# sidiso/surfh

Measured on AMD Instinct MI355X. Metric: CG-iterations/sec (forward+adjoint) on 251x251x4000 cube, higher is better.
Workload: dtype f32 (storage and accumulation; products as 2-piece fp16 splits -- 3 products per fp32 product, 1 on the far tails of the spectral response -- on the 16-bit matrix cores, in the spectral-blur GEMM and in the DFT passes)

## Files before the change

### include/surfh_amd.h

```cpp
#ifndef SURFH_AMD_H
#define SURFH_AMD_H

#include <stdint.h>

#ifdef __cplusplus
extern "C" {
#endif

typedef struct surfh_plan surfh_plan;

typedef struct {
    int32_t wslice_start, wslice_stop;
    int32_t n_pointings;
    int32_t n_slit;
    int32_t n_lambda_out;
    int32_t n_alpha_out;
    int32_t srf;
    int32_t na, nb;
    int32_t alpha0;
    int32_t n_alpha_slit;
    int32_t n_beta_slit;
    const int32_t *slit_beta0;
    const double *slit_weights;
    const int32_t *grid_i0;
    const int32_t *grid_i1;
    const double *grid_y0;
    const double *grid_y1;
    const double *wpsf;
    const int32_t *gt_i0;
    const int32_t *gt_i1;
    const double *gt_y0;
    const double *gt_y1;
    const uint8_t *gt_inside;
    int32_t box_len, box_shift;
} surfh_channel_desc;

typedef struct {
    int32_t n_alpha, n_beta;
    int32_t n_lambda;
    int32_t n_templates;
    const double *templates;
    const double *sotf;
    int32_t n_channels;
    const surfh_channel_desc *channels;
    int32_t device;
    void *stream;
    int32_t split_k_forward;
    int32_t verify;
    int32_t exact;
} surfh_config;

const char *surfh_last_error(void);
int surfh_version(void);

int surfh_plan_create(const surfh_config *cfg, surfh_plan **out);
int surfh_plan_destroy(surfh_plan *plan);

int64_t surfh_isize(const surfh_plan *plan);
int64_t surfh_osize(const surfh_plan *plan);
void *surfh_stream(const surfh_plan *plan);

int surfh_forward(surfh_plan *plan, const float *maps, float *y);
int surfh_adjoint(surfh_plan *plan, const float *y, float *maps);
int surfh_adjoint_ref(surfh_plan *plan, const float *y, float *maps);
int surfh_fwadj(surfh_plan *plan, const float *x, float *out);

int surfh_forward_dev(surfh_plan *plan, const float *maps_dev, float *y_dev);
int surfh_adjoint_dev(surfh_plan *plan, const float *y_dev, float *maps_dev);
int surfh_adjoint_ref_dev(surfh_plan *plan, const float *y_dev, float *maps_dev);
int surfh_fwadj_dev(surfh_plan *plan, const float *x_dev, float *out_dev);

int surfh_wct_forward(surfh_plan *plan, const float *maps, float *cube);
int surfh_wct_adjoint(surfh_plan *plan, const float *cube, float *maps);
int surfh_wct_fwadj(surfh_plan *plan, const float *x, float *out);
int surfh_wct_expsol(surfh_plan *plan, const float *cube, const double *mu_reg, const double *reg_freq, float *maps);

int surfh_cg(surfh_plan *plan, const float *y, double mu, double mu_reg, const float *x0,
             int32_t max_iter, double tol, int32_t refresh, float *x, double *grad_norm, int32_t *nit);
typedef int (*surfh_cg_callback)(void *user, int32_t it, const double *grad_norm, const float *x);
int surfh_cg_cb(surfh_plan *plan, const float *y, double mu, double mu_reg, const float *x0,
                int32_t max_iter, double tol, int32_t refresh, float *x, double *grad_norm, int32_t *nit,
                surfh_cg_callback callback, void *user);
int surfh_mmmg(surfh_plan *plan, const float *y, double mu, double mu_reg, const float *x0,
               int32_t max_iter, double tol, int32_t refresh, float *x, double *grad_norm, int32_t *nit,
               surfh_cg_callback callback, void *user);

int surfh_maps_to_cube(surfh_plan *plan, const double *templates, int32_t n_templates, int32_t n_lambda,
                       const float *maps, float *cube);
int surfh_cube_to_maps(surfh_plan *plan, const double *templates, int32_t n_templates, int32_t n_lambda,
                       const float *cube, float *maps);

int surfh_cg_planes(surfh_plan *plan, const float *y, double mu, double mu_reg, const float *x0, int32_t max_iter,
                    double tol, int32_t refresh, float *x, double *grad_norm, int32_t *nit);
int surfh_mmmg_planes(surfh_plan *plan, const float *y, double mu, double mu_reg, const float *x0, int32_t max_iter,
                      double tol, int32_t refresh, float *x, double *grad_norm, int32_t *nit);

int surfh_cg_planes_begin_dev(surfh_plan *plan, const float *y_dev, double mu, double mu_reg, float *x_dev);
int surfh_cg_planes_step_dev(surfh_plan *plan, int32_t iters, int32_t refresh);
int surfh_cg_planes_rr(surfh_plan *plan, double *rr_host);

int surfh_cg_planes_cb(surfh_plan *plan, const float *y, double mu, double mu_reg, const float *x0, int32_t max_iter,
                       double tol, int32_t refresh, float *x, double *grad_norm, int32_t *nit,
                       surfh_cg_callback callback, void *user);
int surfh_mmmg_planes_cb(surfh_plan *plan, const float *y, double mu, double mu_reg, const float *x0, int32_t max_iter,
                         double tol, int32_t refresh, float *x, double *grad_norm, int32_t *nit,
                         surfh_cg_callback callback, void *user);

int surfh_normal_dev(surfh_plan *plan, const float *d_dev, float *q_dev, double mu);
int surfh_prior_add_dev(surfh_plan *plan, const float *d_dev, float *q_dev, double mu_reg);
int surfh_spec_supported(surfh_plan *plan);
int64_t surfh_spec_size(surfh_plan *plan);
int surfh_to_spec_dev(surfh_plan *plan, const float *x_dev, float *xt_dev);
int surfh_from_spec_dev(surfh_plan *plan, const float *xt_dev, float *x_dev);
int surfh_forward_spec_dev(surfh_plan *plan, const float *dt_dev, float *y_dev);
int surfh_adjoint_spec_dev(surfh_plan *plan, const float *y_dev, float *qt_dev, double mu, const float *dt_dev, double mu_reg);
int surfh_normal_spec_dev(surfh_plan *plan, const float *dt_dev, float *qt_dev, double mu, double mu_reg);
int surfh_prior_spec_add_dev(surfh_plan *plan, const float *dt_dev, float *qt_dev, double mu_reg);
int surfh_set_prior(surfh_plan *plan, int32_t kind);
int surfh_dot_dev(surfh_plan *plan, const float *a_dev, const float *b_dev, int64_t n, double *out_host);
int surfh_cg_step_dev(surfh_plan *plan, float *x_dev, float *r_dev, const float *d_dev,
                      const float *q_dev, int64_t n, double rr_in, double *rr_out_host);
int surfh_cg_dir_dev(surfh_plan *plan, float *d_dev, const float *r_dev, int64_t n, double beta);
int surfh_cg_iter_dev(surfh_plan *plan, float *x_dev, float *r_dev, float *d_dev, const float *q_dev, int64_t n,
                      double rr_in, double *rr_out);

int surfh_cg_begin_dev(surfh_plan *plan, const float *r_dev, int64_t n);
int surfh_cg_iter_nosync_dev(surfh_plan *plan, float *x_dev, float *r_dev, float *d_dev, const float *q_dev, int64_t n);
int surfh_cg_xupdate_nosync_dev(surfh_plan *plan, float *x_dev, const float *d_dev, const float *q_dev, int64_t n);
int surfh_cg_refresh_nosync_dev(surfh_plan *plan, float *r_dev, const float *b_dev, const float *q_dev, float *d_dev, int64_t n);
int32_t surfh_cg_trace(surfh_plan *plan, double *out_host, int32_t capacity);
int surfh_residual_dev(surfh_plan *plan, float *r_dev, const float *b_dev, const float *q_dev, int64_t n);

int surfh_profile_enable(surfh_plan *plan, int32_t on);
int surfh_profile_filter(surfh_plan *plan, const char *prefix);
int32_t surfh_profile_count(surfh_plan *plan);
int surfh_profile_get(surfh_plan *plan, int32_t i, const char **name, int64_t *launches, double *ms);
int surfh_profile_reset(surfh_plan *plan);

int64_t surfh_debug_copy(surfh_plan *plan, const char *which, float *out, int64_t capacity);
int surfh_debug_dims(surfh_plan *plan, const char *which, int64_t dims[4]);

int surfh_gemm_selftest(int32_t device, int32_t M, int32_t N, int32_t K, int32_t split_k,
                        const float *A, const float *B, float *C);
int surfh_gemm_selftest_ksteps(int64_t near_far[2]);
int32_t surfh_klist_classify(const float *B, int32_t n, int32_t k, int64_t ldb, int32_t perm_p, int32_t perm_lin,
                             int32_t *records, int64_t capacity);

typedef struct surfh_tst surfh_tst;
int surfh_tst_create(int32_t n_alpha, int32_t n_beta, int32_t n_lambda, int32_t n_templates, const double *templates,
                     const int32_t *voxels, int64_t n_voxels, const float *S, int32_t device, surfh_tst **out);
int surfh_tst_destroy(surfh_tst *t);
int surfh_tst_forward(surfh_tst *t, const float *maps, float *cube);
int surfh_tst_adjoint(surfh_tst *t, const float *cube, float *maps);
int surfh_tst_fwadj(surfh_tst *t, const float *maps, float *out);
const char *surfh_tst_last_error(void);

int surfh_shepard(int32_t n_seg, const int64_t *pt_off, const float *pt_alpha, const float *pt_lambda,
                  const float *pt_value, const int32_t *n_alpha, const int32_t *n_lambda, int32_t separable,
                  const float *q_alpha, const float *q_lambda, const float *inv_alpha_res, const float *inv_lambda_res,
                  float p, float alpha, float pixel_cutoff, float epsilon, float *out, int32_t *neighbours,
                  int32_t device_ptrs, void *stream, float *kernel_ms);
const char *surfh_shepard_last_error(void);

#ifdef __cplusplus
}
#endif
#endif
```

### surfh_amd/_lib.py

```python
from __future__ import annotations

import ctypes as C
import os

import numpy as np

_HERE = os.path.dirname(os.path.abspath(__file__))
LIB_PATH = os.path.join(_HERE, "libsurfh_amd.so")

c_float_p = C.POINTER(C.c_float)
c_double_p = C.POINTER(C.c_double)
c_int32_p = C.POINTER(C.c_int32)
CG_CALLBACK = C.CFUNCTYPE(C.c_int, C.c_void_p, C.c_int32, c_double_p, c_float_p)
c_uint8_p = C.POINTER(C.c_uint8)


class ChannelDesc(C.Structure):
    _fields_ = [
        ("wslice_start", C.c_int32), ("wslice_stop", C.c_int32),
        ("n_pointings", C.c_int32), ("n_slit", C.c_int32), ("n_lambda_out", C.c_int32),
        ("n_alpha_out", C.c_int32), ("srf", C.c_int32), ("na", C.c_int32), ("nb", C.c_int32),
        ("alpha0", C.c_int32), ("n_alpha_slit", C.c_int32), ("n_beta_slit", C.c_int32),
        ("slit_beta0", c_int32_p), ("slit_weights", c_double_p),
        ("grid_i0", c_int32_p), ("grid_i1", c_int32_p), ("grid_y0", c_double_p), ("grid_y1", c_double_p),
        ("wpsf", c_double_p),
        ("gt_i0", c_int32_p), ("gt_i1", c_int32_p), ("gt_y0", c_double_p), ("gt_y1", c_double_p),
        ("gt_inside", c_uint8_p),
        ("box_len", C.c_int32), ("box_shift", C.c_int32),
    ]


class Config(C.Structure):
    _fields_ = [
        ("n_alpha", C.c_int32), ("n_beta", C.c_int32), ("n_lambda", C.c_int32), ("n_templates", C.c_int32),
        ("templates", c_double_p), ("sotf", c_double_p),
        ("n_channels", C.c_int32), ("channels", C.POINTER(ChannelDesc)),
        ("device", C.c_int32), ("stream", C.c_void_p), ("split_k_forward", C.c_int32), ("verify", C.c_int32),
        ("exact", C.c_int32),
    ]


EXPORTS = [
    "surfh_last_error", "surfh_version", "surfh_plan_create", "surfh_plan_destroy", "surfh_isize", "surfh_osize",
    "surfh_stream", "surfh_forward", "surfh_adjoint", "surfh_adjoint_ref", "surfh_fwadj", "surfh_forward_dev",
    "surfh_adjoint_dev", "surfh_adjoint_ref_dev", "surfh_fwadj_dev", "surfh_wct_forward", "surfh_wct_adjoint",
    "surfh_wct_fwadj", "surfh_wct_expsol", "surfh_tst_create", "surfh_tst_destroy", "surfh_tst_forward",
    "surfh_tst_adjoint", "surfh_tst_fwadj", "surfh_tst_last_error", "surfh_cg", "surfh_cg_cb", "surfh_mmmg", "surfh_cg_planes", "surfh_mmmg_planes", "surfh_cg_planes_cb", "surfh_mmmg_planes_cb", "surfh_cg_planes_begin_dev", "surfh_cg_planes_step_dev", "surfh_cg_planes_rr", "surfh_maps_to_cube", "surfh_cube_to_maps", "surfh_normal_dev",
    "surfh_prior_add_dev", "surfh_spec_supported", "surfh_spec_size", "surfh_to_spec_dev", "surfh_from_spec_dev", "surfh_forward_spec_dev",
    "surfh_adjoint_spec_dev", "surfh_normal_spec_dev", "surfh_prior_spec_add_dev", "surfh_set_prior", "surfh_dot_dev", "surfh_cg_step_dev", "surfh_cg_dir_dev", "surfh_cg_iter_dev", "surfh_residual_dev",
    "surfh_cg_begin_dev", "surfh_cg_iter_nosync_dev", "surfh_cg_xupdate_nosync_dev", "surfh_cg_refresh_nosync_dev", "surfh_cg_trace",
    "surfh_profile_enable", "surfh_profile_filter", "surfh_profile_count", "surfh_profile_get", "surfh_profile_reset", "surfh_debug_copy",
    "surfh_debug_dims", "surfh_gemm_selftest", "surfh_gemm_selftest_ksteps", "surfh_klist_classify",
    "surfh_shepard", "surfh_shepard_last_error",
]

_lib = None


def load():
    global _lib
    if _lib is not None:
        return _lib
    if not os.path.exists(LIB_PATH):
        raise RuntimeError(f"{LIB_PATH} not found: run `python -c 'import __graft_entry__ as g; g.build()'` "
                           "(the HIP path has no CPU fallback)")
    L = C.CDLL(LIB_PATH)
    vp = C.c_void_p
    L.surfh_last_error.restype = C.c_char_p
    L.surfh_version.restype = C.c_int
    L.surfh_plan_create.argtypes = [C.POINTER(Config), C.POINTER(vp)]
    L.surfh_plan_destroy.argtypes = [vp]
    L.surfh_isize.argtypes = [vp]; L.surfh_isize.restype = C.c_int64
    L.surfh_osize.argtypes = [vp]; L.surfh_osize.restype = C.c_int64
    L.surfh_stream.argtypes = [vp]; L.surfh_stream.restype = vp
    for n in ("surfh_forward", "surfh_adjoint", "surfh_adjoint_ref", "surfh_fwadj", "surfh_wct_forward", "surfh_wct_adjoint",
              "surfh_wct_fwadj"):
        getattr(L, n).argtypes = [vp, c_float_p, c_float_p]
    for n in ("surfh_forward_dev", "surfh_adjoint_dev", "surfh_adjoint_ref_dev", "surfh_fwadj_dev"):
        getattr(L, n).argtypes = [vp, vp, vp]
    L.surfh_cg.argtypes = [vp, c_float_p, C.c_double, C.c_double, c_float_p, C.c_int32, C.c_double, C.c_int32,
                           c_float_p, c_double_p, c_int32_p]
    L.surfh_tst_create.argtypes = [C.c_int32] * 4 + [c_double_p, c_int32_p, C.c_int64, c_float_p, C.c_int32, C.POINTER(vp)]
    L.surfh_tst_destroy.argtypes = [vp]
    for n in ("surfh_tst_forward", "surfh_tst_adjoint", "surfh_tst_fwadj"):
        getattr(L, n).argtypes = [vp, c_float_p, c_float_p]
    L.surfh_tst_last_error.restype = C.c_char_p
    L.surfh_wct_expsol.argtypes = [vp, c_float_p, c_double_p, c_double_p, c_float_p]
    L.surfh_cg_planes.argtypes = [vp, c_float_p, C.c_double, C.c_double, c_float_p, C.c_int32, C.c_double, C.c_int32,
                                  c_float_p, c_double_p, c_int32_p]
    L.surfh_cg_cb.argtypes = [vp, c_float_p, C.c_double, C.c_double, c_float_p, C.c_int32, C.c_double, C.c_int32,
                              c_float_p, c_double_p, c_int32_p, CG_CALLBACK, vp]
    L.surfh_mmmg.argtypes = L.surfh_cg_cb.argtypes
    L.surfh_mmmg_planes.argtypes = L.surfh_cg_planes.argtypes
    L.surfh_cg_planes_begin_dev.argtypes = [vp, vp, C.c_double, C.c_double, vp]
    L.surfh_cg_planes_step_dev.argtypes = [vp, C.c_int32, C.c_int32]
    L.surfh_cg_planes_rr.argtypes = [vp, c_double_p]
    L.surfh_cg_planes_cb.argtypes = L.surfh_cg_cb.argtypes
    L.surfh_mmmg_planes_cb.argtypes = L.surfh_cg_cb.argtypes
    L.surfh_maps_to_cube.argtypes = [vp, c_double_p, C.c_int32, C.c_int32, c_float_p, c_float_p]
    L.surfh_cube_to_maps.argtypes = [vp, c_double_p, C.c_int32, C.c_int32, c_float_p, c_float_p]
    L.surfh_normal_dev.argtypes = [vp, vp, vp, C.c_double]
    L.surfh_prior_add_dev.argtypes = [vp, vp, vp, C.c_double]
    L.surfh_spec_supported.argtypes = [vp]
    L.surfh_spec_size.argtypes = [vp]
    L.surfh_spec_size.restype = C.c_int64
    L.surfh_to_spec_dev.argtypes = [vp, vp, vp]
    L.surfh_from_spec_dev.argtypes = [vp, vp, vp]
    L.surfh_forward_spec_dev.argtypes = [vp, vp, vp]
    L.surfh_adjoint_spec_dev.argtypes = [vp, vp, vp, C.c_double, vp, C.c_double]
    L.surfh_normal_spec_dev.argtypes = [vp, vp, vp, C.c_double, C.c_double]
    L.surfh_prior_spec_add_dev.argtypes = [vp, vp, vp, C.c_double]
    L.surfh_set_prior.argtypes = [vp, C.c_int32]
    L.surfh_dot_dev.argtypes = [vp, vp, vp, C.c_int64, c_double_p]
    L.surfh_cg_step_dev.argtypes = [vp, vp, vp, vp, vp, C.c_int64, C.c_double, c_double_p]
    L.surfh_cg_dir_dev.argtypes = [vp, vp, vp, C.c_int64, C.c_double]
    L.surfh_cg_iter_dev.argtypes = [vp, vp, vp, vp, vp, C.c_int64, C.c_double, c_double_p]
    L.surfh_residual_dev.argtypes = [vp, vp, vp, vp, C.c_int64]
    L.surfh_cg_begin_dev.argtypes = [vp, vp, C.c_int64]
    L.surfh_cg_iter_nosync_dev.argtypes = [vp, vp, vp, vp, vp, C.c_int64]
    L.surfh_cg_xupdate_nosync_dev.argtypes = [vp, vp, vp, vp, C.c_int64]
    L.surfh_cg_refresh_nosync_dev.argtypes = [vp, vp, vp, vp, vp, C.c_int64]
    L.surfh_cg_trace.argtypes = [vp, c_double_p, C.c_int32]; L.surfh_cg_trace.restype = C.c_int32
    L.surfh_profile_enable.argtypes = [vp, C.c_int32]
    L.surfh_profile_filter.argtypes = [vp, C.c_char_p]
    L.surfh_profile_count.argtypes = [vp]; L.surfh_profile_count.restype = C.c_int32
    L.surfh_profile_get.argtypes = [vp, C.c_int32, C.POINTER(C.c_char_p), C.POINTER(C.c_int64), c_double_p]
    L.surfh_profile_reset.argtypes = [vp]
    L.surfh_debug_copy.argtypes = [vp, C.c_char_p, c_float_p, C.c_int64]; L.surfh_debug_copy.restype = C.c_int64
    L.surfh_debug_dims.argtypes = [vp, C.c_char_p, C.POINTER(C.c_int64)]
    L.surfh_gemm_selftest.argtypes = [C.c_int32] * 5 + [c_float_p, c_float_p, c_float_p]
    L.surfh_gemm_selftest_ksteps.argtypes = [C.POINTER(C.c_int64)]
    L.surfh_klist_classify.argtypes = [c_float_p, C.c_int32, C.c_int32, C.c_int64, C.c_int32, C.c_int32, C.POINTER(C.c_int32), C.c_int64]
    L.surfh_klist_classify.restype = C.c_int32
    L.surfh_shepard.argtypes = [C.c_int32, C.POINTER(C.c_int64), vp, vp, vp, c_int32_p, c_int32_p, C.c_int32, vp, vp,
                                c_float_p, c_float_p, C.c_float, C.c_float, C.c_float, C.c_float, vp, vp, C.c_int32, vp,
                                c_float_p]
    L.surfh_shepard_last_error.restype = C.c_char_p
    _lib = L
    return L


def check(rc: int, exc=RuntimeError):
    if rc != 0:
        raise exc(load().surfh_last_error().decode("utf-8", "replace"))


def solve(model, fn, data, mu, mu_reg, x0, max_iter, tol, refresh, callback, planes=1, squeeze=True):
    y = np.ascontiguousarray(np.asarray(data, dtype=np.float32).reshape(-1))
    if y.size != model.osize:
        raise ValueError("data size mismatch")
    x0a = None if x0 is None else np.ascontiguousarray(np.asarray(x0, dtype=np.float32).reshape(-1))
    if x0a is not None and x0a.size != model.isize:
        raise ValueError("x0 size mismatch")
    x = np.empty(model.isize, dtype=np.float32)
    gn = np.zeros((max_iter + 1, planes), dtype=np.float64)
    nit = C.c_int32()
    err = []

    def tramp(_user, it, gptr, xptr):
        try:
            g = np.ctypeslib.as_array(gptr, shape=(it + 1, planes)).copy()
            xi = np.ctypeslib.as_array(xptr, shape=(model.isize,)).astype(np.float64).reshape(model.ishape)
            return 1 if callback(it, g[:, 0] if squeeze else g, xi) else 0
        except BaseException as e:
            err.append(e)
            return 1

    cb = CG_CALLBACK(tramp) if callback is not None else CG_CALLBACK()
    check(fn(model._plan, fptr(y), float(mu), float(mu_reg), fptr(x0a) if x0a is not None else None, int(max_iter),
             float(tol), int(refresh), fptr(x), dptr(gn), C.byref(nit), cb, None))
    if err:
        raise err[0]
    gn = gn[: nit.value + 1]
    return x.astype(np.float64).reshape(model.ishape), (gn[:, 0] if squeeze else gn).copy(), nit.value


def fptr(a: np.ndarray):
    return a.ctypes.data_as(c_float_p)


def dptr(a: np.ndarray):
    return a.ctypes.data_as(c_double_p)


def iptr(a: np.ndarray):
    return a.ctypes.data_as(c_int32_p)


def u8ptr(a: np.ndarray):
    return a.ctypes.data_as(c_uint8_p)
```

### surfh_amd/csrc/gemm_cc16.hip

```cpp
#include "gemm_f32.h"
#include "lds_attr.h"
#include <cmath>
#include <cstdlib>
#include <type_traits>

typedef float f32x16 __attribute__((ext_vector_type(16)));
typedef _Float16 f16x8 __attribute__((ext_vector_type(8)));
typedef _Float16 f16x4 __attribute__((ext_vector_type(4)));

namespace {

constexpr int BM = 256, BN = 256, BK = 32;
constexpr int ROWS = BM + BN;
constexpr int PIECE = ROWS * BK;
constexpr int STAGE = 2 * PIECE;
constexpr size_t LDS_BYTES = (size_t)2 * STAGE * sizeof(unsigned short);

__device__ __forceinline__ float f16x2_scale_of(float amax) {
    if (!(amax > 0.f)) return 1.f;
    const int e = (int)((__float_as_uint(amax) >> 23) & 0xFF) - 127;
    int s = e - 13;
    s = s < -126 ? -126 : (s > 127 ? 127 : s);
    return __uint_as_float((unsigned)(s + 127) << 23);
}

__global__ __launch_bounds__(256) void split_rows2h_kernel(const float *__restrict__ src, const unsigned *__restrict__ rowmax,
                                                           unsigned short *__restrict__ dst, int ld, long plane) {
    const int row = blockIdx.y;
    const float inv = 1.f / f16x2_scale_of(__uint_as_float(rowmax[row]));
    const int k4 = (blockIdx.x * 256 + threadIdx.x) * 4;
    if (k4 >= ld) return;
    const long o = (long)row * ld + k4;
    const float4 v = *reinterpret_cast<const float4 *>(src + o);
    const float x0 = v.x * inv, x1 = v.y * inv, x2 = v.z * inv, x3 = v.w * inv;
    const _Float16 h0 = (_Float16)x0, h1 = (_Float16)x1, h2 = (_Float16)x2, h3 = (_Float16)x3;
    f16x4 h = {h0, h1, h2, h3};
    f16x4 l = {(_Float16)(x0 - (float)h0), (_Float16)(x1 - (float)h1), (_Float16)(x2 - (float)h2), (_Float16)(x3 - (float)h3)};
    *reinterpret_cast<f16x4 *>(dst + o) = h;
    *reinterpret_cast<f16x4 *>(dst + plane + o) = l;
}

#ifndef CC_EXP
#define CC_EXP 0
#endif
constexpr int CC2_MAXSEG = 64;
constexpr size_t LDS2_BYTES = LDS_BYTES + (size_t)CC2_MAXSEG * BM;

__device__ __forceinline__ const char *cc2_uniform(const char *p) {
    const unsigned long long v = (unsigned long long)p;
    const unsigned lo = __builtin_amdgcn_readfirstlane((unsigned)v), hi = __builtin_amdgcn_readfirstlane((unsigned)(v >> 32));
    return (const char *)(((unsigned long long)hi << 32) | lo);
}
__device__ __forceinline__ int cc2_seg_of(int k, int segLinP, int segChunks) {
    const int col = k / segLinP, in = k % segLinP;
    return __builtin_amdgcn_readfirstlane(col * segChunks + in / 1024);
}
__device__ __forceinline__ int cc2_seg_end(int k, int segLinP) {
    const int col = k / segLinP, in = k % segLinP;
    const int e1 = col * segLinP + (in / 1024 + 1) * 1024, e2 = (col + 1) * segLinP;
    return __builtin_amdgcn_readfirstlane(e1 < e2 ? e1 : e2);
}
__device__ __forceinline__ float cc2_pow2_ratio(unsigned eo, unsigned en) {
    int e = (int)eo - (int)en + 127;
    e = e < 1 ? 1 : (e > 254 ? 254 : e);
    return __uint_as_float((unsigned)e << 23);
}
__device__ __forceinline__ void cc2_dma(const char *base, unsigned off, unsigned l) {
    asm volatile("s_mov_b32 m0, %2\n\ts_nop 0\n\tglobal_load_lds_dwordx4 %0, %1" ::"v"(off), "s"(base), "s"(l) : "memory");
}

#define CC_MFMA_DRAIN() asm volatile("s_nop 15\n\ts_nop 15\n\ts_nop 7" ::: "memory")

typedef float f32x4v __attribute__((ext_vector_type(4)));

template <int U, int N, bool DMA, bool FAR>
__device__ __forceinline__ void cc16_slot(f32x4v (&acc)[4][8], f16x8 (&A)[4][2], const f16x8 (&Bc)[2][2], f16x8 (&Bn)[2][2], unsigned ran,
                                          unsigned rbn, const char *ka, const char *kb, long pA2, long pB2, const unsigned (&offA)[2],
                                          const unsigned (&offB)[2], unsigned ls) {
    constexpr int i = N / 6, jj = (N / 3) & 1, j = 2 * U + jj, p = N % 3;
    if constexpr (!(CC_EXP & 4) && (!FAR || p == 2))
        asm volatile("v_mfma_f32_16x16x32_f16 %0, %1, %2, %0" : "+v"(acc[i][j]) : "v"(A[i][p == 0 ? 1 : 0]), "v"(Bc[jj][p == 1 ? 1 : 0]));
    if constexpr (N < 4 && !(CC_EXP & 2)) {
        constexpr int jn = 2 * ((U + 1) & 3) + (N >> 1), q = N & 1;
        if constexpr (!FAR || q == 0)
            asm volatile("ds_read_b128 %0, %1 offset:%2" : "=v"(Bn[N >> 1][q]) : "v"(rbn), "n"(q * PIECE * 2 + jn * 16 * BK * 2));
    }
    if constexpr (U == 3 && N % 6 == 5 && !(CC_EXP & 2)) {
        asm volatile("ds_read_b128 %0, %1 offset:%2" : "=v"(A[i][0]) : "v"(ran), "n"(i * 16 * BK * 2));
        if constexpr (!FAR) asm volatile("ds_read_b128 %0, %1 offset:%2" : "=v"(A[i][1]) : "v"(ran), "n"(PIECE * 2 + i * 16 * BK * 2));
    }
    constexpr int d = (U == 3 && N % 3 != 2 && N < 12) ? N - N / 3 : -1;
    if constexpr (DMA && d >= 0 && !(CC_EXP & 1) && (!FAR || d < 4)) {
        constexpr int q = d >> 2, i2 = (d >> 1) & 1;
        if constexpr (d & 1) cc2_dma(kb + q * pB2, offB[i2], ls + (unsigned)((q * PIECE + (BM + i2 * 128) * BK) * 2));
        else cc2_dma(ka + q * pA2, offA[i2], ls + (unsigned)((q * PIECE + i2 * 128 * BK) * 2));
    }
}
template <int U, bool DMA, bool FAR, int N = 0>
__device__ __forceinline__ void cc16_unit(f32x4v (&acc)[4][8], f16x8 (&A)[4][2], const f16x8 (&Bc)[2][2], f16x8 (&Bn)[2][2], unsigned ran,
                                          unsigned rbn, const char *ka, const char *kb, long pA2, long pB2, const unsigned (&offA)[2],
                                          const unsigned (&offB)[2], unsigned ls) {
    if constexpr (N < 24) {
        if constexpr (U == 0 && N == 18 && !(CC_EXP & 2)) {
            if constexpr (FAR) asm volatile("s_waitcnt lgkmcnt(3)" : "+v"(A[3][0]), "+v"(A[3][1]));
            else asm volatile("s_waitcnt lgkmcnt(5)" : "+v"(A[3][0]), "+v"(A[3][1]));
        }
        cc16_slot<U, N, DMA, FAR>(acc, A, Bc, Bn, ran, rbn, ka, kb, pA2, pB2, offA, offB, ls);
        cc16_unit<U, DMA, FAR, N + 1>(acc, A, Bc, Bn, ran, rbn, ka, kb, pA2, pB2, offA, offB, ls);
    }
}
#define CC16_WAITB(n_, B_)                                                                                              \
    asm volatile("s_waitcnt lgkmcnt(" #n_ ")" : "+v"(B_[0][0]), "+v"(B_[1][0]), "+v"(B_[0][1]), "+v"(B_[1][1]))

constexpr int CC2_MAXLIST = 2048;
constexpr size_t LDS3_BYTES = LDS2_BYTES + (size_t)CC2_MAXLIST * sizeof(int);

struct GemmGroup {
    GemmArgs g[GEMM_GROUP_MAX];
    long first[GEMM_GROUP_MAX + 1];
    int n;
};

__global__ __launch_bounds__(512, 1) void gemm_nt_f16x2_cc_kernel(GemmGroup grp) {
    extern __shared__ __attribute__((aligned(16))) unsigned short lds[];
    const long gtotal = grp.first[grp.n], per = (gtotal + 7) / 8;
    const long vg = (long)(blockIdx.x & 7) * per + (blockIdx.x >> 3);
    if ((long)(blockIdx.x >> 3) >= per || vg >= gtotal) return;
    int gi = 0;
    while (gi + 1 < grp.n && vg >= grp.first[gi + 1]) ++gi;
    const long v = vg - grp.first[gi];
    const GemmArgs g = grp.g[gi];
    unsigned char *sctab = reinterpret_cast<unsigned char *>(lds + 2 * STAGE);
    int *klds = reinterpret_cast<int *>(sctab + CC2_MAXSEG * BM);
    const int tid = threadIdx.x, lane = tid & 63, wave = __builtin_amdgcn_readfirstlane(tid >> 6);
    const int Q = g.permP ? BN / g.permP : BN, tilesL = g.permP ? g.permLin / Q : 0, ncol = g.permP ? g.N / g.permLin : 0;
    const int tilesM = (g.M + BM - 1) / BM, tilesN = g.permP ? (ncol + g.permP - 1) / g.permP * tilesL : (g.N + BN - 1) / BN, tiles = tilesM * tilesN;
    auto bcol = [&](int tn_, int v) __attribute__((always_inline)) {
        if (!g.permP) { const int n = tn_ * BN + v; return n < g.N ? n : -1; }
        const int c = (tn_ / tilesL) * g.permP + v / Q;
        return c < ncol ? c * g.permLin + (tn_ % tilesL) * Q + v % Q : -1;
    };
    const int t = (int)(v % tiles), z = (int)(v / tiles);
    const int tm = t % tilesM, tn = t / tilesM;
    const int b = z / g.splitK, sk = z % g.splitK;
    const int m0 = tm * BM;
    const float *bs = g.bscale;

    int nnear, nfar, seg0 = 0, nseg = 0;
    if (g.klist) {
        const int *kl = g.klist + (long)tn * g.klistStride;
        const int NN = kl[0], NF = kl[1];
        const int a0 = (int)((long)NN * sk / g.splitK), a1 = (int)((long)NN * (sk + 1) / g.splitK);
        const int f0 = (int)((long)NF * sk / g.splitK), f1 = (int)((long)NF * (sk + 1) / g.splitK);
        nnear = __builtin_amdgcn_readfirstlane(a1 - a0);
        nfar = __builtin_amdgcn_readfirstlane(f1 - f0);
        for (int e = tid; e < nnear; e += 512) klds[e] = kl[2 + a0 + e];
        for (int e = tid; e < nfar; e += 512) klds[nnear + e] = kl[2 + NN + f0 + e];
        if (bs) nseg = (g.K / g.segLinP) * g.segChunks;
    } else {
        const int Kper = g.K / g.splitK, kbeg = sk * Kper;
        nnear = Kper / BK;
        nfar = 0;
        if (bs) {
            seg0 = cc2_seg_of(kbeg, g.segLinP, g.segChunks);
            nseg = cc2_seg_of(kbeg + Kper - 1, g.segLinP, g.segChunks) - seg0 + 1;
        }
        for (int e = tid; e < nnear; e += 512) {
            const int k = kbeg + e * BK;
            klds[e] = (k / BK) | (bs ? ((k / g.segLinP) * g.segChunks + (k % g.segLinP) / 1024) << 16 : 0);
        }
    }
    for (int e = tid; e < nseg * BM; e += 512) {
        int row = m0 + (e & (BM - 1));
        row = row < g.M ? row : g.M - 1;
        sctab[e] = (unsigned char)(__float_as_uint(bs[(long)(seg0 + (e >> 8)) * g.M + row]) >> 23);
    }

    unsigned offA[2], offB[2];
    {
        const int chunk = (lane & 3) ^ ((-(lane >> 4)) & 3);
#pragma unroll
        for (int i = 0; i < 2; ++i) {
            int m = m0 + (wave + 8 * i) * 16 + (lane >> 2);
            m = m < g.M ? m : g.M - 1;
            offA[i] = (unsigned)(((long)m * g.lda + 8 * chunk) * 2);
            int n = bcol(tn, (wave + 8 * i) * 16 + (lane >> 2));
            n = n >= 0 ? n : g.N - 1;
            offB[i] = (unsigned)(((long)n * g.ldb + 8 * chunk) * 2);
        }
    }
    const char *baseA = cc2_uniform(reinterpret_cast<const char *>(g.A3 + (long)b * g.sA));
    const char *baseB = cc2_uniform(reinterpret_cast<const char *>(g.B16 + (long)b * g.sB));
    const long pA2 = g.pA3 * 2, pB2 = g.pB16 * 2;
    const unsigned ldsw = (unsigned)(size_t)lds + (unsigned)(wave * 16 * BK * 2);
    const unsigned kaddr = (unsigned)(size_t)klds;
    const int l15 = lane & 15, kc = lane >> 4;
    const int wm = wave >> 1, wn = wave & 1;
    f32x4v acc[4][8];
#pragma unroll
    for (int i = 0; i < 4; ++i)
#pragma unroll
        for (int j = 0; j < 8; ++j) acc[i][j] = f32x4v{0.f, 0.f, 0.f, 0.f};
    const unsigned ra0 = (unsigned)(size_t)lds + (unsigned)(((wm * 64 + l15) * BK + ((kc ^ ((-(l15 >> 2)) & 3)) * 8)) * 2);
    const unsigned fbd = (unsigned)((BM + wn * 128 - wm * 64) * BK * 2);
    const bool active = m0 + wm * 64 < g.M;
    const int srow = wm * 64 + 4 * kc;
    int seg = -1;

    f16x8 A[4][2], Bx[2][2], By[2][2];
#define CC_RD(dst_, addr_, off_) asm volatile("ds_read_b128 %0, %1 offset:%2" : "=v"(dst_) : "v"(addr_), "n"(off_))
#define CC_DMA(FAR_, ks_, st_)                                                                                         \
    {                                                                                                                  \
        const char *ka = baseA + (long)(ks_) * (BK * 2), *kb = baseB + (long)(ks_) * (BK * 2);                         \
        const unsigned ls = ldsw + stofs((FAR_), (st_));                                                               \
        _Pragma("unroll") for (int q = 0; q < ((FAR_) ? 1 : 2); ++q) {                                                 \
            _Pragma("unroll") for (int i = 0; i < 2; ++i) {                                                            \
                cc2_dma(ka + q * pA2, offA[i], ls + (q * PIECE + i * 128 * BK) * 2);                                   \
                cc2_dma(kb + q * pB2, offB[i], ls + (q * PIECE + (BM + i * 128) * BK) * 2);                            \
            }                                                                                                          \
        }                                                                                                              \
    }
    auto stofs = [](bool far, int s) __attribute__((always_inline)) {
        return far ? (unsigned)((s >> 1) * (STAGE * 2) + (s & 1) * (PIECE * 2)) : (unsigned)(s * (STAGE * 2));
    };
    __syncthreads();

    auto kloop = [&](auto far_tag, const int lb, const int n) __attribute__((always_inline)) {
        constexpr bool FAR = decltype(far_tag)::value;
        constexpr int D = FAR ? 4 : 2;
        if (n <= 0) return;
        int e[D];
#pragma unroll
        for (int s = 0; s < D; ++s) {
            e[s] = __builtin_amdgcn_readfirstlane(klds[lb + (s < n ? s : n - 1)]);
            CC_DMA(FAR, e[s] & 0xFFFF, s);
        }
        if (FAR) asm volatile("s_waitcnt vmcnt(12)" ::: "memory");
        else asm volatile("s_waitcnt vmcnt(8)" ::: "memory");
        __syncthreads();
        if (!active) {
            for (int kt = 0; kt < n; ++kt) {
                if (FAR) asm volatile("s_waitcnt vmcnt(8)\n\ts_barrier" ::: "memory");
                else asm volatile("s_waitcnt vmcnt(0)\n\ts_barrier" ::: "memory");
                const int ed = __builtin_amdgcn_readfirstlane(klds[lb + (kt + D < n ? kt + D : n - 1)]);
                CC_DMA(FAR, ed & 0xFFFF, kt & (D - 1));
            }
            asm volatile("s_waitcnt vmcnt(0)" ::: "memory");
            return;
        }
        unsigned ra = ra0, rb = ra0 + fbd;
        if (!(CC_EXP & 2)) {
#pragma unroll
            for (int i = 0; i < 4; ++i) {
                CC_RD(A[i][0], ra, 0 + 0);
                if (!FAR) CC_RD(A[i][1], ra, PIECE * 2);
                ra += 16 * BK * 2;
            }
            ra -= 4 * 16 * BK * 2;
            CC_RD(Bx[0][0], rb, 0); CC_RD(Bx[1][0], rb, 16 * BK * 2);
            if (!FAR) { CC_RD(Bx[0][1], rb, PIECE * 2); CC_RD(Bx[1][1], rb, PIECE * 2 + 16 * BK * 2); }
            asm volatile("s_waitcnt lgkmcnt(0)" : "+v"(A[0][0]), "+v"(A[0][1]), "+v"(A[1][0]), "+v"(A[1][1]), "+v"(A[2][0]), "+v"(A[2][1]), "+v"(A[3][0]),
                         "+v"(A[3][1]), "+v"(Bx[0][0]), "+v"(Bx[1][0]), "+v"(Bx[0][1]), "+v"(Bx[1][1]));
        }
        for (int kt = 0; kt < n; ++kt) {
            const int nseg_ = e[0] >> 16;
            if (bs && nseg_ != seg) {
                if (seg >= 0) {
                    const unsigned char *to = sctab + (seg - seg0) * BM + srow, *tn_ = sctab + (nseg_ - seg0) * BM + srow;
                    unsigned so[4], sn[4];
                    bool same = true;
#pragma unroll
                    for (int i = 0; i < 4; ++i) {
                        so[i] = *reinterpret_cast<const unsigned *>(to + i * 16);
                        sn[i] = *reinterpret_cast<const unsigned *>(tn_ + i * 16);
                        same = same && so[i] == sn[i];
                    }
                    if (__builtin_amdgcn_ballot_w64(!same) != 0ull) {
                        CC_MFMA_DRAIN();
#pragma unroll
                        for (int i = 0; i < 4; ++i) {
                            const f32x4v rt = {cc2_pow2_ratio(so[i] & 255u, sn[i] & 255u), cc2_pow2_ratio((so[i] >> 8) & 255u, (sn[i] >> 8) & 255u),
                                               cc2_pow2_ratio((so[i] >> 16) & 255u, (sn[i] >> 16) & 255u), cc2_pow2_ratio(so[i] >> 24, sn[i] >> 24)};
#pragma unroll
                            for (int j = 0; j < 8; ++j) acc[i][j] *= rt;
                            __builtin_amdgcn_sched_barrier(0);
                        }
                    }
                }
                seg = nseg_;
            }
            unsigned ev;
            asm volatile("ds_read_b32 %0, %1" : "=v"(ev) : "v"(kaddr + 4u * (unsigned)(lb + (kt + D < n ? kt + D : n - 1))));
            const char *kz = baseA;
            const unsigned ls2 = ldsw + stofs(FAR, kt & (D - 1));
            cc16_unit<0, false, FAR>(acc, A, Bx, By, ra, rb, kz, kz, pA2, pB2, offA, offB, ls2);
            asm volatile("s_waitcnt lgkmcnt(0)" : "+v"(By[0][0]), "+v"(By[1][0]), "+v"(By[0][1]), "+v"(By[1][1]), "+v"(ev));
            const int en = __builtin_amdgcn_readfirstlane((int)ev);
            const char *ka2 = baseA + (long)(en & 0xFFFF) * (BK * 2), *kb2 = baseB + (long)(en & 0xFFFF) * (BK * 2);
            cc16_unit<1, false, FAR>(acc, A, By, Bx, ra, rb, kz, kz, pA2, pB2, offA, offB, ls2);
            CC16_WAITB(0, Bx);
            cc16_unit<2, false, FAR>(acc, A, Bx, By, ra, rb, kz, kz, pA2, pB2, offA, offB, ls2);
            CC16_WAITB(0, By);
            if (FAR) asm volatile("s_waitcnt vmcnt(8)\n\ts_barrier" ::: "memory");
            else asm volatile("s_waitcnt vmcnt(0)\n\ts_barrier" ::: "memory");
            {
                const unsigned nx = stofs(FAR, (kt + 1) & (D - 1));
                ra = ra0 + nx; rb = ra0 + fbd + nx;
            }
            cc16_unit<3, true, FAR>(acc, A, By, Bx, ra, rb, ka2, kb2, pA2, pB2, offA, offB, ls2);
            if (FAR) { CC16_WAITB(1, Bx); }
            else { CC16_WAITB(2, Bx); }
#pragma unroll
            for (int s = 0; s + 1 < D; ++s) e[s] = e[s + 1];
            e[D - 1] = en;
        }
        asm volatile("s_waitcnt vmcnt(0) lgkmcnt(0)" ::: "memory");
    };
    kloop(std::false_type{}, 0, nnear);
    if (nfar > 0) {
        __syncthreads();
        kloop(std::true_type{}, nnear, nfar);
    }
    if (!active) return;
    CC_MFMA_DRAIN();
#undef CC_DMA
#undef CC_RD
    {
        char *Cb = reinterpret_cast<char *>(g.C + (long)b * g.sC + (long)sk * g.sCsplit + (long)m0 * g.ldc);
        int cj[8];
#pragma unroll
        for (int j = 0; j < 8; ++j) {
            const int c0 = bcol(tn, wn * 128 + j * 16);
            cj[j] = c0 >= 0 ? c0 + l15 : -1;
        }
        const unsigned ldc4 = (unsigned)(g.ldc * 4);
#pragma unroll
        for (int i = 0; i < 4; ++i) {
            float rsc[4];
#pragma unroll
            for (int r = 0; r < 4; ++r) {
                const int lr = srow + i * 16 + r;
                int row = m0 + lr;
                row = row < g.M ? row : g.M - 1;
                rsc[r] = bs ? (seg >= 0 ? __uint_as_float((unsigned)sctab[(seg - seg0) * BM + lr] << 23) : 1.f) : f16x2_scale_of(__uint_as_float(g.amax[(long)b * g.M + row]));
            }
#pragma unroll
            for (int r = 0; r < 4; ++r) {
                const int row = m0 + srow + i * 16 + r;
                const float sc = rsc[r] * g.sB16;
                const unsigned o_ = (unsigned)(srow + i * 16 + r) * ldc4;
#pragma unroll
                for (int j = 0; j < 8; ++j)
                    if (row < g.M && cj[j] >= 0 && cj[j] < g.N) *reinterpret_cast<float *>(Cb + (o_ + (unsigned)cj[j] * 4u)) = acc[i][j][r] * sc;
            }
        }
    }
}
#undef CC16_WAITB

__global__ __launch_bounds__(256) void split2h_kernel(const float *__restrict__ src, unsigned short *__restrict__ dst, long n4, long plane,
                                                      float inv) {
    const long stride = (long)gridDim.x * 256;
    for (long i = (long)blockIdx.x * 256 + threadIdx.x; i < n4; i += stride) {
        const float4 v = reinterpret_cast<const float4 *>(src)[i];
        const float x0 = v.x * inv, x1 = v.y * inv, x2 = v.z * inv, x3 = v.w * inv;
        const _Float16 h0 = (_Float16)x0, h1 = (_Float16)x1, h2 = (_Float16)x2, h3 = (_Float16)x3;
        f16x4 h = {h0, h1, h2, h3};
        f16x4 l = {(_Float16)(x0 - (float)h0), (_Float16)(x1 - (float)h1), (_Float16)(x2 - (float)h2), (_Float16)(x3 - (float)h3)};
        *reinterpret_cast<f16x4 *>(dst + 4 * i) = h;
        *reinterpret_cast<f16x4 *>(dst + plane + 4 * i) = l;
    }
}

}

float gemm_f16x2_scale(float amax) {
    if (!(amax > 0.f)) return 1.f;
    int e = 0;
    std::frexp(amax, &e);
    int s = (e - 1) - 13;
    s = s < -126 ? -126 : (s > 127 ? 127 : s);
    return std::ldexp(1.f, s);
}

int launch_split2h(hipStream_t stream, const float *src, unsigned short *dst2, long n, long plane, float scale) {
    if (n % 4 || plane % 4 || !(scale > 0.f)) return (int)hipErrorInvalidValue;
    const long n4 = n / 4;
    long nb = (n4 + 255) / 256;
    hipLaunchKernelGGL(split2h_kernel, dim3((unsigned)(nb > 4096 ? 4096 : (nb < 1 ? 1 : nb))), dim3(256), 0, stream, src, dst2, n4, plane,
                       1.f / scale);
    return (int)hipGetLastError();
}

int launch_split_rows2h(hipStream_t stream, const float *src, const unsigned *rowmax, unsigned short *dst2, int rows, int ld, long plane) {
    if (ld % 4 || plane % 4 || rows < 1) return (int)hipErrorInvalidValue;
    hipLaunchKernelGGL(split_rows2h_kernel, dim3((ld / 4 + 255) / 256, rows), dim3(256), 0, stream, src, rowmax, dst2, ld, plane);
    return (int)hipGetLastError();
}

static int check_gemm_nt_f16x2_cc(const GemmArgs &g, long *items) {
    if (g.M % 64 || g.N % 128 || g.K % (BK * g.splitK) || g.splitK < 1 || g.batch < 1 || g.accumulate || g.lda % 8 || g.ldb % 8 || !g.A3 ||
        !g.B16 || g.pA3 % 8 || g.pB16 % 8 || (!g.amax && !g.bscale) || !(g.sB16 > 0.f))
        return (int)hipErrorInvalidValue;
    if (g.bscale && (g.batch != 1 || g.segLinP < BK || g.segLinP % BK || g.segChunks != (g.segLinP + 1023) / 1024 || g.K % g.segLinP))
        return (int)hipErrorInvalidValue;
    if ((double)(BM + 1) * (double)g.ldc * 4.0 >= 2147483648.0) return (int)hipErrorInvalidValue;
    if ((double)g.M * (double)g.lda * 2.0 >= 4294967296.0 || (double)g.N * (double)g.ldb * 2.0 >= 4294967296.0) return (int)hipErrorInvalidValue;
    if (g.klist) {
        if (g.batch != 1 || g.klistStride < 2 + g.K / BK || g.K / BK > CC2_MAXLIST || g.K / BK > 0xFFFF) return (int)hipErrorInvalidValue;
        if (g.bscale && (g.K / g.segLinP) * g.segChunks > CC2_MAXSEG) return (int)hipErrorInvalidValue;
    } else {
        const int Kper = g.K / g.splitK;
        if (Kper / BK > CC2_MAXLIST || g.K / BK > 0xFFFF) return (int)hipErrorInvalidValue;
        if (g.bscale) {
            auto seg_of = [&](int k) { return (k / g.segLinP) * g.segChunks + (k % g.segLinP) / 1024; };
            for (int sk = 0; sk < g.splitK; ++sk)
                if (seg_of(sk * Kper + Kper - 1) - seg_of(sk * Kper) + 1 > CC2_MAXSEG) return (int)hipErrorInvalidValue;
        }
    }
    long tilesN = (g.N + BN - 1) / BN;
    if (g.permP) {
        if ((g.permP != 1 && g.permP != 2 && g.permP != 4 && g.permP != 8) || g.permLin < 1 || g.permLin % (BN / g.permP) || g.N % g.permLin)
            return (int)hipErrorInvalidValue;
        tilesN = (long)((g.N / g.permLin + g.permP - 1) / g.permP) * (g.permLin / (BN / g.permP));
    }
    *items = (long)((g.M + BM - 1) / BM) * tilesN * g.batch * g.splitK;
    return 0;
}

int launch_gemm_nt_f16x2_cc_group(hipStream_t stream, const GemmArgs *gs, int n) {
    if (n < 1 || n > GEMM_GROUP_MAX) return (int)hipErrorInvalidValue;
    GemmGroup grp;
    grp.n = n;
    grp.first[0] = 0;
    for (int i = 0; i < n; ++i) {
        long items = 0;
        if (int e = check_gemm_nt_f16x2_cc(gs[i], &items)) return e;
        grp.g[i] = gs[i];
        grp.first[i + 1] = grp.first[i] + items;
    }
    for (int i = n; i < GEMM_GROUP_MAX; ++i) grp.first[i + 1] = grp.first[n];
    const long total = grp.first[n];
    if (total >= 2147483647L - 8) return (int)hipErrorInvalidValue;
    dim3 grid((unsigned)(8 * ((total + 7) / 8)));
    static unsigned long long attr_done = 0;
    if (int e = ensure_dynamic_lds(gemm_nt_f16x2_cc_kernel, LDS3_BYTES, attr_done)) return e;
    hipLaunchKernelGGL(gemm_nt_f16x2_cc_kernel, grid, dim3(512), LDS3_BYTES, stream, grp);
    return (int)hipGetLastError();
}

int launch_gemm_nt_f16x2_cc(hipStream_t stream, const GemmArgs &g) { return launch_gemm_nt_f16x2_cc_group(stream, &g, 1); }
```

### surfh_amd/csrc/gemm_f32.h

```cpp
#pragma once
#include <hip/hip_runtime.h>
#include <stdint.h>

struct GemmArgs {
    const float *A0 = nullptr, *A1 = nullptr;
    int ksplitA = 1 << 30;
    long lda = 0, sA = 0;
    const float *B0 = nullptr, *B1 = nullptr;
    int ksplitB = 1 << 30;
    long ldb = 0, sB = 0;
    float *C = nullptr;
    long ldc = 0, sC = 0;
    int M = 0, N = 0, K = 0;
    int batch = 1;
    int splitK = 1;
    long sCsplit = 0;
    int accumulate = 0;
    const unsigned short *A3 = nullptr, *B16 = nullptr;
    long pA3 = 0, pB16 = 0;
    float sB16 = 0.f;
    const unsigned *amax = nullptr;
    const float *bscale = nullptr;
    int segLinP = 0, segChunks = 0;
    const int *klist = nullptr;
    int klistStride = 0;
    int permP = 0, permLin = 0;
};

int launch_gemm_f32(hipStream_t stream, const GemmArgs &g);
int launch_gemm_f64acc(hipStream_t stream, const GemmArgs &g);

int launch_split2h(hipStream_t stream, const float *src, unsigned short *dst2, long n, long plane, float scale);
float gemm_f16x2_scale(float amax);
int launch_gemm_nt_f16x2_cc(hipStream_t stream, const GemmArgs &g);
constexpr int GEMM_GROUP_MAX = 4;
int launch_gemm_nt_f16x2_cc_group(hipStream_t stream, const GemmArgs *g, int n);
int launch_split_rows2h(hipStream_t stream, const float *src, const unsigned *rowmax, unsigned short *dst2, int rows, int ld, long plane);
```

### surfh_amd/csrc/plan.hip

```cpp
#include <hip/hip_runtime.h>

#include <algorithm>
#include <array>
#include <cmath>
#include <cstdarg>
#include <cstdio>
#include <cstring>
#include <map>
#include <string>
#include <vector>

#include "../../include/surfh_amd.h"
#include "dft_h2.h"
#include "dft_ct.h"
#include "gemm_f32.h"
#include "kernels.h"

namespace {

thread_local std::string g_err;

int fail(const char *fmt, ...) {
    char buf[1024];
    va_list ap;
    va_start(ap, fmt);
    vsnprintf(buf, sizeof buf, fmt, ap);
    va_end(ap);
    g_err = buf;
    return 1;
}

#define HIP_OK(expr)                                                                              \
    do {                                                                                          \
        hipError_t e_ = (expr);                                                                   \
        if (e_ != hipSuccess) return fail("%s failed: %s (%s:%d)", #expr, hipGetErrorString(e_), __FILE__, __LINE__); \
    } while (0)
#define LAUNCH_OK(expr)                                                                           \
    do {                                                                                          \
        int e_ = (expr);                                                                          \
        if (e_ != 0) return fail("%s failed: %s (%s:%d)", #expr, hipGetErrorString((hipError_t)e_), __FILE__, __LINE__); \
    } while (0)

inline int pad64(int n) { return (n + 63) / 64 * 64; }

struct HostEll {
    std::vector<std::vector<std::pair<int64_t, float>>> rows;
    std::vector<int64_t> dst;
};

struct DevEll {
    EllTable t;
    int32_t *cnt = nullptr;
    int64_t *col = nullptr, *dst = nullptr;
    float *val = nullptr;
    uint32_t *rmw = nullptr;
    int2 *rng = nullptr, *g_rng = nullptr;
    std::vector<int64_t> host_dst;
    GroupTable g;
    int32_t *g_cnt = nullptr;
    int64_t *g_col = nullptr, *g_dst = nullptr;
    float *g_val = nullptr;
    uint32_t *g_rmw = nullptr;
};

struct Channel {
    int ws0 = 0, ws1 = 0, Lin = 0, P = 0, S = 0, Ldet = 0, aout = 0, srf = 0, na = 0, nb = 0, alpha0 = 0, nas = 0,
        nbs = 0;
    int ws0a = 0;
    int LinA = 0;
    int LinP = 0;
    int shift = 0;
    int nlam = 0;
    int K = 0, NP = 0, LdetP = 0, splitK = 1;
    long yoff = 0, ysize = 0;
    float *W = nullptr, *Wt = nullptr, *Xs = nullptr, *Cpart = nullptr, *ymat = nullptr;
    unsigned short *W16 = nullptr, *Wt16 = nullptr;
    unsigned short *Xs16 = nullptr, *ymat16 = nullptr;
    float *bscale = nullptr;
    float sW = 1.f;
    int *klF = nullptr, *klA = nullptr;
    int klFs = 0, klAs = 0;
    int permA = 0;
    long ksteps[4] = {0, 0, 0, 0};
    unsigned *amax = nullptr;
    unsigned *pmax = nullptr;
    DevEll fwd, adjT, adjRef;
    HostEll adjT_host;
    bool has_ref = false;
    bool bsum = false;
};

struct ProfRec {
    const char *name;
    hipEvent_t a, b;
};

}

struct surfh_plan {
    int dev = 0;
    hipStream_t stream = nullptr;
    bool own_stream = false;
    hipStream_t stream2 = nullptr;
    bool overlap = false;
    std::vector<hipEvent_t> sync_ev;
    size_t sync_next = 0;
    int Na = 0, Nb = 0, Lc = 0, T = 0, NAP = 0, NBP = 0, KAP = 0, KBP = 0;
    long PL = 0, PLc = 0;
    int lo = 0, hi = 0, Lown = 0, LP = 0;
    struct Seg { int start, len, coff; };
    std::vector<Seg> segs;
    std::vector<int> planes;
    int compact(int l) const {
        for (auto &g : segs) if (l >= g.start && l <= g.start + g.len) return g.coff + (l - g.start);
        return -1;
    }
    float *sotf = nullptr, *tpl = nullptr, *mhat = nullptr, *spec = nullptr, *ycol = nullptr, *cube = nullptr,
          *maps_pad = nullptr, *ycol_maps = nullptr;
    float *Fi = nullptr, *Gi = nullptr, *Gf = nullptr, *Ff = nullptr, *GiT = nullptr, *GfT = nullptr;
    float *Cma = nullptr, *Sma = nullptr, *Gc = nullptr, *Gs = nullptr, *Cf = nullptr, *Sf = nullptr;
    int MPa = 0, KPa = 0, MPb = 0, KPb = 0;
    int n_cu = 256;
    bool gather_sorted = true;
    bool gemm_grouped = true;
    bool scatter_grouped = true;
    bool otf_prod = true;
    bool gather_grouped = true;
    bool dense_dft = false, fuse_mix = true, wblur_fp32 = false;
    bool verify = false;
    int prior_kind = 0;
    bool h2 = false;
    unsigned short *h2img = nullptr;
    bool ct = false, ilv = false;
    DftCtPlan ctA, ctB;
    int ax_a = 0, ax_b = 0;
    int a_lo = 0, a_hi = 0, b_lo = 0, b_hi = 0;
    float *ycol_adj = nullptr;
    const float *spec_in = nullptr;
    float *spec_out = nullptr;
    const float *spec_prior_src = nullptr;
    float spec_mu = 1.f, spec_prior_mu = 0.f;
    float *adjmix_part = nullptr;
    int *otf_vlist = nullptr, *otf_kbstart = nullptr;
    int otf_nvalid = 0;
    int *otf_tabs = nullptr;
    float *ycol_mix = nullptr;
    int h2kA[3] = {0, 0, 0};
    float *io_x = nullptr, *io_y = nullptr, *io_cube = nullptr, *hth = nullptr, *mhat2 = nullptr;
    float *gcube = nullptr;
    std::vector<Channel> ch;
    long isize = 0, osize = 0;
    float *cg_x = nullptr, *cg_r = nullptr, *cg_d = nullptr, *cg_q = nullptr, *cg_b = nullptr, *cg_y = nullptr, *cg_qm = nullptr, *cg_dd = nullptr;
    double *dscal = nullptr, *dscratch = nullptr;
    double *cg_hist = nullptr;
    int cg_hist_n = 0;
    double *pl_sc = nullptr;
    float *pl_x = nullptr;
    double pl_mu = 1.0, pl_mu_reg = 0.0;
    int pl_it = 0;
    float *pn_v[5] = {nullptr, nullptr, nullptr, nullptr, nullptr};
    double *pn_sc = nullptr, *pn_part = nullptr;
    bool pn_native = false, pn_active = false, pn_fold_prior = false;
    bool prof = false;
    std::string prof_filter;
    std::vector<ProfRec> pending;
    std::vector<hipEvent_t> pool;
    std::map<std::string, std::pair<long, double>> acc;
    std::vector<std::string> acc_names;
};

namespace {

struct Prof {
    surfh_plan *p;
    ProfRec r;
    bool on;
    hipStream_t st;
    Prof(surfh_plan *pl, const char *name, hipStream_t stream = nullptr) : p(pl), on(pl->prof), st(stream ? stream : pl->stream) {
        if (on && !pl->prof_filter.empty() && strncmp(name, pl->prof_filter.c_str(), pl->prof_filter.size()) != 0) on = false;
        if (!on) return;
        r.name = name;
        for (hipEvent_t *e : {&r.a, &r.b}) {
            if (!p->pool.empty()) {
                *e = p->pool.back();
                p->pool.pop_back();
            } else {
                hipEventCreate(e);
            }
        }
        hipEventRecord(r.a, st);
    }
    ~Prof() {
        if (!on) return;
        hipEventRecord(r.b, st);
        p->pending.push_back(r);
    }
};

int chain(surfh_plan *p, hipStream_t from, hipStream_t to) {
    if (from == to) return 0;
    if (p->sync_next == p->sync_ev.size()) {
        hipEvent_t e;
        HIP_OK(hipEventCreateWithFlags(&e, hipEventDisableTiming));
        p->sync_ev.push_back(e);
    }
    hipEvent_t e = p->sync_ev[p->sync_next++];
    if (p->sync_next >= 64) p->sync_next = 0;
    HIP_OK(hipEventRecord(e, from));
    HIP_OK(hipStreamWaitEvent(to, e, 0));
    return 0;
}

void prof_collect(surfh_plan *p) {
    if (p->pending.empty()) return;
    hipStreamSynchronize(p->stream);
    if (p->stream2) hipStreamSynchronize(p->stream2);
    for (auto &r : p->pending) {
        float ms = 0.f;
        hipEventElapsedTime(&ms, r.a, r.b);
        auto &e = p->acc[r.name];
        e.first += 1;
        e.second += ms;
        p->pool.push_back(r.a);
        p->pool.push_back(r.b);
    }
    p->pending.clear();
    p->acc_names.clear();
    for (auto &kv : p->acc) p->acc_names.push_back(kv.first);
}

template <typename Tp>
int dev_alloc(Tp **p, size_t n) {
    HIP_OK(hipMalloc((void **)p, std::max<size_t>(n, 1) * sizeof(Tp)));
    return 0;
// ... 147 lines not shown

    const int64_t LP = p->LP;
    auto pix_off = [&](int ia, int ib) -> int64_t { return ((int64_t)ib * p->NAP + ia) * LP + c->ws0a; };
    auto xs_off = [&](int pt, int s, int a, int b) -> int64_t {
        return ((int64_t)((pt * c->S + s) * c->aout + a)) * c->K + (c->bsum ? 0 : (int64_t)b * c->LinP);
    };

    HostEll f;
    std::vector<std::vector<std::pair<int, int>>> colslit(c->nb);
    for (int s = 0; s < c->S; ++s)
        for (int b = 0; b < c->nbs; ++b) colslit[d.slit_beta0[s] + b].push_back({s, b});
    for (int pt = 0; pt < c->P; ++pt)
        for (int a = 0; a < c->aout; ++a)
            for (int j = 0; j < c->nb; ++j)
                for (auto &sb : colslit[j]) {
                    const int s = sb.first, b = sb.second;
                    const double ws = d.slit_weights[(long)s * c->nbs + b];
                    std::vector<std::pair<int64_t, float>> row;
                    std::map<int64_t, double> acc;
                    for (int r = 0; r < box; ++r) {
                        const int i = (c->alpha0 + a * c->srf + r + bsh + c->na) % c->na;
                        const long li = (long)pt * nloc + (long)i * c->nb + j;
                        const int i0 = d.grid_i0[li], i1 = d.grid_i1[li];
                        const double y0 = d.grid_y0[li], y1 = d.grid_y1[li];
                        const double w[4] = {(1. - y0) * (1. - y1), (1. - y0) * y1, y0 * (1. - y1), y0 * y1};
                        const int da[4] = {0, 0, 1, 1}, db[4] = {0, 1, 0, 1};
                        for (int k = 0; k < 4; ++k)
                            if (w[k] * ws != 0.0) acc[pix_off(i0 + da[k], i1 + db[k])] += w[k] * ws;
                    }
                    for (auto &e : acc) row.push_back({e.first, (float)e.second});
                    f.rows.push_back(std::move(row));
                    f.dst.push_back(xs_off(pt, s, a, b));
                }
    if (c->bsum) {
        std::map<int64_t, std::map<int64_t, double>> mg;
        for (size_t r = 0; r < f.rows.size(); ++r)
            for (auto &e : f.rows[r]) mg[f.dst[r]][e.first] += (double)e.second;
        HostEll f2;
        for (auto &row : mg) {
            std::vector<std::pair<int64_t, float>> v;
            for (auto &e : row.second) v.push_back({e.first, (float)e.second});
            f2.rows.push_back(std::move(v));
            f2.dst.push_back(row.first);
        }
        f = std::move(f2);
    }
    if (p->gather_sorted) {
        std::vector<size_t> ord(f.rows.size());
        for (size_t i = 0; i < ord.size(); ++i) ord[i] = i;
        std::stable_sort(ord.begin(), ord.end(), [&](size_t a, size_t b) {
            const int64_t ka = f.rows[a].empty() ? INT64_MAX : f.rows[a][0].first, kb = f.rows[b].empty() ? INT64_MAX : f.rows[b][0].first;
            return ka < kb;
        });
        HostEll g;
        g.rows.reserve(ord.size());
        g.dst.reserve(ord.size());
        for (size_t i : ord) {
            g.rows.push_back(std::move(f.rows[i]));
            g.dst.push_back(f.dst[i]);
        }
        f = std::move(g);
    }
    if (upload_ell(f, &c->fwd)) return 1;
    if (p->gather_grouped && p->gather_sorted && !c->bsum) {
        std::vector<std::pair<size_t, size_t>> runs;
        for (size_t r = 0; r < f.rows.size(); r += GATHER_G) runs.push_back({r, std::min<size_t>(GATHER_G, f.rows.size() - r)});
        if (upload_groups(f, runs, nullptr, &c->fwd, GATHER_G)) return 1;
    }

    {
        std::map<int64_t, std::map<int64_t, double>> tr;
        for (size_t r = 0; r < f.rows.size(); ++r)
            for (auto &e : f.rows[r]) tr[e.first][f.dst[r]] += (double)e.second;
        HostEll t;
        for (auto &px : tr) {
            std::vector<std::pair<int64_t, float>> row;
            for (auto &e : px.second) row.push_back({e.first, (float)e.second});
            t.rows.push_back(std::move(row));
            t.dst.push_back(px.first);
        }
        if (upload_ell(t, &c->adjT)) return 1;
        for (int64_t o : t.dst) {
            const int ia = (int)((o / LP) % p->NAP), ib = (int)((o / LP) / p->NAP);
            p->a_lo = std::min(p->a_lo, ia); p->a_hi = std::max(p->a_hi, ia + 1);
            p->b_lo = std::min(p->b_lo, ib); p->b_hi = std::max(p->b_hi, ib + 1);
        }
        c->adjT.host_dst = t.dst;
        c->adjT_host = std::move(t);
    }

    c->has_ref = d.gt_i0 && d.gt_i1 && d.gt_y0 && d.gt_y1 && d.gt_inside;
    if (c->has_ref) {
        std::vector<std::vector<int>> arow(c->na);
        for (int a = 0; a < c->aout; ++a)
            for (int r = 0; r < box; ++r) arow[(c->alpha0 + a * c->srf + r + bsh + c->na) % c->na].push_back(a);
        HostEll t;
        const long npix = (long)p->Na * p->Nb;
        for (int ib = 0; ib < p->Nb; ++ib)
            for (int ia = 0; ia < p->Na; ++ia) {
                std::map<int64_t, double> m;
                for (int pt = 0; pt < c->P; ++pt) {
                    const long gi = (long)pt * npix + (long)ia * p->Nb + ib;
                    if (!d.gt_inside[gi]) continue;
                    const int i0 = d.gt_i0[gi], i1 = d.gt_i1[gi];
                    if (i0 < 0 || i0 > c->na - 2 || i1 < 0 || i1 > c->nb - 2) return fail("gridding_t index out of range");
                    const double y0 = d.gt_y0[gi], y1 = d.gt_y1[gi];
                    const double w[4] = {(1. - y0) * (1. - y1), (1. - y0) * y1, y0 * (1. - y1), y0 * y1};
                    const int li[4] = {i0, i0, i0 + 1, i0 + 1}, lj[4] = {i1, i1 + 1, i1, i1 + 1};
                    for (int k = 0; k < 4; ++k)
                        if (w[k] != 0.0)
                        for (int a : arow[li[k]])
                            for (auto &sb : colslit[lj[k]])
                                m[xs_off(pt, sb.first, a, sb.second)] += w[k] * d.slit_weights[(long)sb.first * c->nbs + sb.second];
                }
                if (m.empty()) continue;
                std::vector<std::pair<int64_t, float>> row;
                for (auto &e : m) row.push_back({e.first, (float)e.second});
                t.rows.push_back(std::move(row));
                t.dst.push_back(pix_off(ia, ib));
            }
        if (upload_ell(t, &c->adjRef)) return 1;
        for (int64_t o : t.dst) {
            const int ia = (int)((o / LP) % p->NAP), ib = (int)((o / LP) / p->NAP);
            p->a_lo = std::min(p->a_lo, ia); p->a_hi = std::max(p->a_hi, ia + 1);
            p->b_lo = std::min(p->b_lo, ib); p->b_hi = std::max(p->b_hi, ib + 1);
        }
    }

    if (!c->bsum) {
        std::vector<float> W((size_t)c->LdetP * c->K, 0.f), Wt((size_t)c->K * c->LdetP, 0.f);
        for (int l = 0; l < c->Ldet; ++l)
            for (int lam = 0; lam < c->Lin; ++lam)
                for (int b = 0; b < c->nbs; ++b) {
                    const float v = (float)d.wpsf[((long)l * c->Lin + lam) * c->nbs + b];
                    const size_t k = (size_t)b * c->LinP + c->shift + lam;
                    W[(size_t)l * c->K + k] = v;
                    Wt[k * c->LdetP + l] = v;
                }
        float wmax = 0.f;
        for (float v : W) wmax = std::max(wmax, std::fabs(v));
        c->sW = gemm_f16x2_scale(wmax);
        if (dev_upload(&c->W, W) || dev_upload(&c->Wt, Wt)) return 1;
    }
    if (dev_alloc(&c->Xs, (size_t)c->NP * c->K)) return 1;
    HIP_OK(hipMemset(c->Xs, 0, (size_t)c->NP * c->K * sizeof(float)));
    if (!c->bsum) {
        if (dev_alloc(&c->ymat, (size_t)c->NP * c->LdetP)) return 1;
        HIP_OK(hipMemset(c->ymat, 0, (size_t)c->NP * c->LdetP * sizeof(float)));
    }
    return 0;
}

int build_klist(const float *B, int N, int K, long ldb, int segLinP, int segChunks, double tol1, double tol2, std::vector<int> *out,
                int *stride, long *n_near, long *n_far, int permP = 0, int permLin = 0) {
    const int Q = permP ? 256 / permP : 256, tilesL = permP ? permLin / Q : 0, ncol = permP ? N / permLin : 0;
    const int nb = K / 32, tilesN = permP ? (ncol + permP - 1) / permP * tilesL : (N + 255) / 256;
    auto brow = [&](int tn, int v) {
        if (!permP) { const int n = tn * 256 + v; return n < N ? n : -1; }
        const int c = (tn / tilesL) * permP + v / Q;
        return c < ncol ? c * permLin + (tn % tilesL) * Q + v % Q : -1;
    };
    *stride = 2 + nb;
    out->assign((size_t)tilesN * *stride, 0);
    *n_near = *n_far = 0;
    std::vector<double> l1((size_t)256 * nb), l2((size_t)256 * nb), L1(256), L2(256), c1(256), c2(256), imp(nb);
    std::vector<int> order(nb);
    std::vector<char> far(nb);
    for (int tn = 0; tn < tilesN; ++tn) {
        const int nr = 256;
        for (int r = 0; r < nr; ++r) {
            const int br = brow(tn, r);
            if (br < 0) {
                for (int b = 0; b < nb; ++b) l1[(size_t)r * nb + b] = l2[(size_t)r * nb + b] = 0.0;
                L1[r] = L2[r] = 0.0;
                continue;
            }
            const float *row = B + (long)br * ldb;
            double s1 = 0.0, s2 = 0.0;
            for (int b = 0; b < nb; ++b) {
                double a1 = 0.0, a2 = 0.0;
                for (int k = 0; k < 32; ++k) { const double v = row[b * 32 + k]; a1 += std::fabs(v); a2 += v * v; }
                l1[(size_t)r * nb + b] = a1; l2[(size_t)r * nb + b] = a2;
                s1 += a1; s2 += a2;
            }
            L1[r] = s1; L2[r] = s2;
        }
        for (int b = 0; b < nb; ++b) {
            double m = 0.0;
            for (int r = 0; r < nr; ++r)
                if (L1[r] > 0.0) m = std::max(m, std::max(l1[(size_t)r * nb + b] / (L1[r] * tol1), std::sqrt(l2[(size_t)r * nb + b] / L2[r]) / tol2));
            imp[b] = m;
            order[b] = b;
            far[b] = 0;
        }
        std::stable_sort(order.begin(), order.end(), [&](int a, int b) { return imp[a] < imp[b]; });
        std::fill(c1.begin(), c1.end(), 0.0);
        std::fill(c2.begin(), c2.end(), 0.0);
        int nf = 0;
        for (int i = 0; i < nb; ++i) {
            const int b = order[i];
            bool ok = true;
            for (int r = 0; r < nr && ok; ++r)
                ok = c1[r] + l1[(size_t)r * nb + b] <= tol1 * L1[r] && c2[r] + l2[(size_t)r * nb + b] <= tol2 * tol2 * L2[r];
            if (!ok) break;
            for (int r = 0; r < nr; ++r) { c1[r] += l1[(size_t)r * nb + b]; c2[r] += l2[(size_t)r * nb + b]; }
            far[b] = 1;
            ++nf;
        }
        if (nf < 8) { std::fill(far.begin(), far.end(), 0); nf = 0; }
        int *rec = out->data() + (size_t)tn * *stride;
        rec[0] = nb - nf; rec[1] = nf;
        int in = 2, ifar = 2 + nb - nf;
        for (int b = 0; b < nb; ++b) {
            const int k = b * 32;
            const int e = b | ((segLinP ? (k / segLinP) * segChunks + (k % segLinP) / 1024 : 0) << 16);
            if (far[b]) rec[ifar++] = e; else rec[in++] = e;
        }
        *n_near += nb - nf; *n_far += nf;
    }
    return 0;
}

int pick_split(const Channel &c, int forced, bool f16, int n_cu) {
    if (forced > 0) return (c.K % (32 * forced) == 0) ? forced : 1;
    if (f16) {
        constexpr int max_steps = 136, tile_m = 256, tile_n = 256;
        const long tiles = (long)((c.NP + tile_m - 1) / tile_m) * ((c.LdetP + tile_n - 1) / tile_n);
        const int steps = c.K / 32;
        int smin = 0;
        for (int s = 1; s <= steps; ++s)
            if (steps % s == 0 && steps / s <= max_steps) { smin = s; break; }
        if (!smin) return 1;
        int best = smin;
        double best_t = -1.0;
        for (int s = smin; s <= steps / 16 && s <= steps; ++s) {
            if (steps % s) continue;
            const double t = (double)((tiles * s + n_cu - 1) / n_cu) * (steps / s) + 3.0 * s;
            if (best_t < 0 || t < best_t) { best_t = t; best = s; }
        }
        return best;
    }
    const int bm = (c.NP % 128 == 0) ? 128 : 64, bn = (c.LdetP % 128 == 0) ? 128 : 64;
    const long tiles = (long)(c.NP / bm) * (c.LdetP / bn);
    int best = 1;
    for (int s : {1, 2, 3, 4, 6, 8, 12, 16, 24, 32}) {
        if (c.K % (32 * s)) continue;
        if (c.K / s < 256) break;
        best = s;
        if (tiles * s >= 768) break;
    }
    return best;
}

void build_dft(const surfh_plan *p, std::vector<float> &Fi, std::vector<float> &Gi, std::vector<float> &Gf,
               std::vector<float> &Ff, std::vector<float> &GiT, std::vector<float> &GfT) {
    const int Na = p->Na, Nb = p->Nb, NAP = p->NAP, NBP = p->NBP, KAP = p->KAP, KBP = p->KBP;
    const int nkb = Nb / 2 + 1;
    const double sa = 1.0 / std::sqrt((double)Na), sb = 1.0 / std::sqrt((double)Nb);
    Fi.assign((size_t)2 * NAP * 2 * KAP, 0.f);
    Ff.assign((size_t)2 * KAP * 2 * NAP, 0.f);
    Gi.assign((size_t)2 * KBP * NBP, 0.f);
    Gf.assign((size_t)NBP * 2 * KBP, 0.f);
    GiT.assign((size_t)NBP * 2 * KBP, 0.f);
    GfT.assign((size_t)2 * KBP * NBP, 0.f);
    for (int a = 0; a < Na; ++a)
        for (int k = 0; k < Na; ++k) {
            const long m = ((long)a * k) % Na;
            const double th = 2.0 * M_PI * (double)m / (double)Na;
            const double c = std::cos(th) * sa, s = std::sin(th) * sa;
            Fi[((size_t)0 * NAP + a) * (2 * KAP) + 0 * KAP + k] = (float)c;
            Fi[((size_t)0 * NAP + a) * (2 * KAP) + 1 * KAP + k] = (float)(-s);
            Fi[((size_t)1 * NAP + a) * (2 * KAP) + 0 * KAP + k] = (float)s;
            Fi[((size_t)1 * NAP + a) * (2 * KAP) + 1 * KAP + k] = (float)c;
            Ff[((size_t)0 * KAP + k) * (2 * NAP) + 0 * NAP + a] = (float)c;
            Ff[((size_t)0 * KAP + k) * (2 * NAP) + 1 * NAP + a] = (float)s;
            Ff[((size_t)1 * KAP + k) * (2 * NAP) + 0 * NAP + a] = (float)(-s);
            Ff[((size_t)1 * KAP + k) * (2 * NAP) + 1 * NAP + a] = (float)c;
        }
    for (int b = 0; b < Nb; ++b)
        for (int k = 0; k < nkb; ++k) {
            const long m = ((long)b * k) % Nb;
            const double th = 2.0 * M_PI * (double)m / (double)Nb;
            const double c = std::cos(th) * sb, s = std::sin(th) * sb;
            const double w = (k == 0 || (Nb % 2 == 0 && k == Nb / 2)) ? 1.0 : 2.0;
            Gi[((size_t)0 * KBP + k) * NBP + b] = (float)(w * c);
            Gi[((size_t)1 * KBP + k) * NBP + b] = (float)(-w * s);
            Gf[(size_t)b * (2 * KBP) + 0 * KBP + k] = (float)c;
            Gf[(size_t)b * (2 * KBP) + 1 * KBP + k] = (float)(-s);
            GiT[(size_t)b * (2 * KBP) + 0 * KBP + k] = (float)(w * c);
            GiT[(size_t)b * (2 * KBP) + 1 * KBP + k] = (float)(-w * s);
            GfT[((size_t)0 * KBP + k) * NBP + b] = (float)c;
            GfT[((size_t)1 * KBP + k) * NBP + b] = (float)(-s);
        }
}

int prior_add(surfh_plan *p, hipStream_t st, const float *d, float *q, int n_img, float mu_reg) {
    return p->prior_kind == 1 ? launch_prior_joint_add(st, d, q, n_img, p->Na, p->Nb, mu_reg) : launch_prior_add(st, d, q, n_img, p->Na, p->Nb, mu_reg);
}

int gemm32(surfh_plan *p, hipStream_t st, const GemmArgs &g) { return p->verify ? launch_gemm_f64acc(st, g) : launch_gemm_f32(st, g); }

int rfft2_planes(surfh_plan *p, const float *src, float *dst, int B) {
    GemmArgs g;
    g.A0 = src; g.lda = p->NBP; g.sA = p->PLc;
    g.B0 = p->Gf; g.ldb = 2 * p->KBP; g.sB = 0;
    g.C = p->ycol_maps; g.ldc = 2 * p->KBP; g.sC = (long)p->NAP * 2 * p->KBP;
    g.M = p->NAP; g.N = 2 * p->KBP; g.K = p->NBP; g.batch = B;
    {
        Prof pr(p, "gemm_dft_rows_fwd_maps");
        LAUNCH_OK(gemm32(p, p->stream, g));
    }
    GemmArgs h;
    h.A0 = p->Ff; h.lda = 2 * p->NAP; h.sA = 0;
    h.B0 = p->ycol_maps; h.B1 = p->ycol_maps + p->KBP; h.ksplitB = p->NAP; h.ldb = 2 * p->KBP;
    h.sB = (long)p->NAP * 2 * p->KBP;
    h.C = dst; h.ldc = p->KBP; h.sC = 2 * p->PL;
    h.M = 2 * p->KAP; h.N = p->KBP; h.K = 2 * p->NAP; h.batch = B;
    {
        Prof pr(p, "gemm_dft_cols_fwd_maps");
        LAUNCH_OK(gemm32(p, p->stream, h));
    }
    return 0;
}

int irfft2_planes(surfh_plan *p, const float *src, float *dst, int B) {
    GemmArgs g;
    g.A0 = p->Fi; g.lda = 2 * p->KAP; g.sA = 0;
    g.B0 = src; g.ldb = p->KBP; g.sB = 2 * p->PL;
    g.C = p->ycol_maps; g.ldc = p->KBP; g.sC = (long)2 * p->NAP * p->KBP;
    g.M = 2 * p->NAP; g.N = p->KBP; g.K = 2 * p->KAP; g.batch = B;
    {
        Prof pr(p, "gemm_dft_cols_inv_maps");
        LAUNCH_OK(gemm32(p, p->stream, g));
    }
    GemmArgs h;
    h.A0 = p->ycol_maps; h.A1 = p->ycol_maps + (long)p->NAP * p->KBP; h.ksplitA = p->KBP; h.lda = p->KBP;
    h.sA = (long)2 * p->NAP * p->KBP;
    h.B0 = p->Gi; h.ldb = p->NBP; h.sB = 0;
    h.C = dst; h.ldc = p->NBP; h.sC = p->PLc;
    h.M = p->NAP; h.N = p->NBP; h.K = 2 * p->KBP; h.batch = B;
    {
        Prof pr(p, "gemm_dft_rows_inv_maps");
        LAUNCH_OK(gemm32(p, p->stream, h));
    }
    return 0;
}

int rfft2_lam(surfh_plan *p, const float *src, float *dst) {
    const long LP = p->LP;
    GemmArgs g;
    g.A0 = p->GfT; g.lda = p->NBP;
    g.B0 = src; g.ldb = p->NAP * LP;
    g.C = p->ycol; g.ldc = p->NAP * LP;
    g.M = 2 * p->KBP; g.N = (int)(p->NAP * LP); g.K = p->NBP;
    {
        Prof pr(p, "gemm_dft_rows_fwd");
        LAUNCH_OK(gemm32(p, p->stream, g));
    }
    GemmArgs h;
    h.A0 = p->Ff; h.lda = 2 * p->NAP;
    h.B0 = p->ycol; h.B1 = p->ycol + (long)p->KBP * p->NAP * LP; h.ksplitB = p->NAP; h.ldb = LP; h.sB = p->NAP * LP;
    h.C = dst; h.ldc = p->KBP * LP; h.sC = LP;
    h.M = 2 * p->KAP; h.N = (int)LP; h.K = 2 * p->NAP; h.batch = p->KBP;
    {
        Prof pr(p, "gemm_dft_cols_fwd");
        LAUNCH_OK(gemm32(p, p->stream, h));
    }
    return 0;
}
// ... 217 lines not shown
    g.dst = p->ycol; g.ldc = 2 * p->KBP * LP;
    g.ncols = (int)(hb * LP); g.batch = 1;
    if (mix) { g.mhat = p->mhat; g.tpl = p->tpl; g.T = p->T; g.LP = (int)p->LP; g.PL = p->PL; g.KBP = p->KBP; }
    if (mix && p->spec_in) { g.mhat = p->spec_in; g.mhat_self = 1.f; g.mhat_pair = 0.70710678118654752f; g.mix_Nb = p->Nb; }
    if (po && po->prod && !mix) {
        g.loader = DFT_CT_PROD; g.prod = po->prod; g.ldp = g.ldb; g.sP = 0; g.prod_sign = po->sign; g.scale *= po->scale;
        if (po->add && po->add_w != 0.f) {
            g.loader = DFT_CT_PRODADD; g.add = po->add; g.add_w = po->add_w; g.add_Nb = p->Nb; g.LP = (int)p->LP;
        }
    }
    const bool supp = mix && p->otf_vlist && p->ycol_mix && p->otf_tabs;
    float *const yc = supp ? p->ycol_mix : p->ycol;
    if (supp) { g.vlist = p->otf_vlist; g.nvalid = p->otf_nvalid; g.dst = yc; g.ktab = p->otf_tabs; g.tabLP = (int)LP; }
    if (which & 2) {
        Prof pr(p, mix ? "dft_ct_cols_inv_mix" : (g.loader == DFT_CT_PROD ? "dft_ct_cols_inv_prod" : g.loader == DFT_CT_PRODADD ? "dft_ct_cols_inv_prodadd" : "dft_ct_cols_inv"));
        LAUNCH_OK(launch_dft_ct(p->stream, g, p->ctA));
    }
    if (!(which & 1)) return 0;
    const bool sub = acols && p->a_hi > p->a_lo;
    const int a0 = sub ? p->a_lo : 0, na = sub ? p->a_hi - p->a_lo : p->Na;
    DftCtArgs h;
    h.R = p->ctB.R; h.M = p->ctB.M; h.loader = DFT_CT_HPACK; h.epi = DFT_CT_STORE; h.sgn = 1.f;
    h.scale = (float)(1.0 / std::sqrt((double)p->Nb));
    h.src = yc + (long)a0 * 2 * p->KBP * LP; h.ldb = 2 * LP; h.sB = 2 * p->KBP * LP;
    h.dst = dst + (long)a0 * LP; h.ldc = p->NAP * LP; h.sC = LP;
    h.ncols = (int)(LP / 2); h.batch = na;
    if (supp) { h.ktab = p->otf_tabs + LP / 128; h.tabLP = (int)(LP / 2); h.tabShift = 6; }
    {
        Prof pr(p, "dft_ct_rows_inv");
        LAUNCH_OK(launch_dft_ct(p->stream, h, p->ctB));
    }
    return 0;
}

int rfft2_lam_ilv(surfh_plan *p, const float *src, float *dst, float *madj = nullptr, bool acols = false, bool lists = false) {
    if (p->h2) return rfft2_lam_h2(p, src, dst, madj, acols);
    if (p->ax_b == 1 ? rfft2_lam_h2(p, src, dst, nullptr, acols, 1) : rfft2_lam_ct(p, src, dst, acols, lists, 1)) return 1;
    return p->ax_a == 1 ? rfft2_lam_h2(p, src, dst, nullptr, acols, 2) : rfft2_lam_ct(p, src, dst, acols, lists, 2);
}
int irfft2_lam_ilv(surfh_plan *p, const float *src, float *dst, bool mix = false, bool acols = false, const ProdOperand *po = nullptr) {
    if (po && p->ax_a != 2) return fail("irfft2: the product loader needs the Cooley-Tukey pass along alpha");
    if (p->h2) return irfft2_lam_h2(p, src, dst, mix, acols);
    if (p->ax_a == 1 ? irfft2_lam_h2(p, src, dst, mix, acols, 2) : irfft2_lam_ct(p, src, dst, mix, acols, 2, po)) return 1;
    return p->ax_b == 1 ? irfft2_lam_h2(p, src, dst, mix, acols, 1) : irfft2_lam_ct(p, src, dst, mix, acols, 1);
}

int rfft2_cube(surfh_plan *p, const float *src, float *dst) { return p->dense_dft ? rfft2_lam(p, src, dst) : rfft2_lam_ilv(p, src, dst); }
int irfft2_cube(surfh_plan *p, const float *src, float *dst, bool mix = false, bool acols = false, const ProdOperand *po = nullptr) {
    if (po && p->dense_dft) return fail("irfft2: the product loader is not part of the dense plan");
    return p->dense_dft ? irfft2_lam(p, src, dst) : irfft2_lam_ilv(p, src, dst, mix, acols, po);
}

int adjoint_tail(surfh_plan *p, const float *cube, bool acols = false) {
    if (p->adjmix_part && p->h2 && p->T > 0) return rfft2_lam_h2(p, cube, p->spec, p->spec_out ? p->spec_out : p->mhat, acols);
    if (p->ct && !p->dense_dft) {
        if (rfft2_lam_ilv(p, cube, p->spec, nullptr, acols, true)) return 1;
        if (prod_capable(p)) return 0;
        SpecmixAdjOpt o;
        o.Na = p->Na; o.KBP = p->KBP;
        if (p->T > 0 && p->otf_vlist && p->ycol_mix && p->otf_tabs) o.lim = p->otf_tabs + 2 * (p->LP / 128);
        if (p->spec_out) {
            o.Nb = p->Nb; o.out_self = p->spec_mu; o.out_pair = p->spec_mu * 1.41421356237309505f;
            o.prior_src = p->spec_prior_src; o.prior_mu = p->spec_prior_mu;
        }
        Prof pr(p, "specmix_adj");
        if (p->T == 0 && p->pn_fold_prior) {
            SpecmixAdjOpt o2;
            o2.Na = p->Na; o2.Nb = p->Nb; o2.KBP = p->KBP; o2.out_self = (float)p->pl_mu; o2.prior_src = p->mhat; o2.prior_mu = (float)p->pl_mu_reg;
            LAUNCH_OK(launch_specmix_adj(p->stream, p->spec, p->sotf, p->tpl, p->mhat, 0, p->PL, p->LP, false, 1, &o2));
            return 0;
        }
        LAUNCH_OK(launch_specmix_adj(p->stream, p->spec, p->sotf, p->tpl, p->spec_out ? p->spec_out : p->mhat, p->T, p->PL, p->LP, false, 1,
                                     p->T > 0 ? &o : nullptr));
        return 0;
    }
    if (rfft2_cube(p, cube, p->spec)) return 1;
    Prof pr(p, "specmix_adj");
    if (p->T == 0 && p->ilv && p->pn_fold_prior) {
        SpecmixAdjOpt o;
        o.Na = p->Na; o.Nb = p->Nb; o.KBP = p->KBP; o.out_self = (float)p->pl_mu; o.prior_src = p->mhat; o.prior_mu = (float)p->pl_mu_reg;
        LAUNCH_OK(launch_specmix_adj(p->stream, p->spec, p->sotf, p->tpl, p->mhat, 0, p->PL, p->LP, false, 1, &o));
        return 0;
    }
    LAUNCH_OK(launch_specmix_adj(p->stream, p->spec, p->sotf, p->tpl, p->mhat, p->T, p->PL, p->LP, p->verify, p->ilv));
    return 0;
}

int forward_dev(surfh_plan *p, const float *x, float *y, bool hand_over = false) {
    hipStream_t s = p->stream;
    if (p->spec_in) {
    } else if (p->T > 0) {
        {
            Prof pr(p, "pad_planes");
            LAUNCH_OK(launch_pad_planes(s, x, p->maps_pad, p->T, p->Na, p->Nb, p->NAP, p->NBP));
        }
        if (rfft2_planes(p, p->maps_pad, p->mhat, p->T)) return 1;
    } else if (p->pn_native) {
        if (rfft2_cube(p, x, p->mhat)) return 1;
    } else {
        {
            Prof pr(p, "cube_transpose");
            for (auto &g : p->segs)
                LAUNCH_OK(launch_cube_to_lam_inner(s, x, p->cube + g.coff, g.start, g.len, p->Na, p->Nb, p->NAP, p->LP));
        }
        if (rfft2_cube(p, p->cube, p->mhat)) return 1;
    }
    if (p->T > 0 && p->T <= 4 && p->fuse_mix && !p->dense_dft) {
        if (irfft2_cube(p, p->sotf, p->cube, true, hand_over)) return 1;
    } else if (prod_capable(p)) {
        ProdOperand po;
        po.prod = p->sotf;
        if (irfft2_cube(p, p->mhat, p->cube, false, false, &po)) return 1;
    } else {
        {
            Prof pr(p, "specmix_fwd");
            LAUNCH_OK(launch_specmix_fwd(s, p->mhat, p->sotf, p->tpl, p->spec, p->T, p->PL, p->LP, p->ilv));
        }
        if (irfft2_cube(p, p->spec, p->cube)) return 1;
    }
    hipStream_t sB = (p->overlap && p->stream2) ? p->stream2 : s;
    for (auto &c : p->ch) {
        const bool f16 = c.W16 != nullptr;
        {
            Prof pr(p, "spmm_gather_fwd");
            if (c.Xs16 && c.fwd.g.NG)
                LAUNCH_OK(launch_spmm_group_gather_f16(s, c.fwd.g, p->cube, c.Xs16, (long)c.NP * c.K, c.nlam, c.bscale, c.NP, c.K, c.LinP));
            else if (c.Xs16)
                LAUNCH_OK(launch_spmm_rows_f16(s, c.fwd.t, p->cube, c.Xs16, (long)c.NP * c.K, c.nlam, c.bscale, c.NP, c.K, c.LinP));
            else if (p->verify)
                LAUNCH_OK(launch_spmm_rows_f64acc(s, c.fwd.t, p->cube, c.Xs, c.nlam, 0));
            else
                LAUNCH_OK(launch_spmm_rows(s, c.fwd.t, p->cube, c.Xs, c.nlam, 0));
        }
        if (c.bsum) {
            Prof pr(p, "y_transpose");
            LAUNCH_OK(launch_cube_from_lam_inner(s, c.Xs + c.shift, y + c.yoff, 0, c.Lin, 1, c.P * c.S * c.aout, 1, c.LinP));
            continue;
        }
        if (chain(p, s, sB)) return 1;
        GemmArgs g;
        g.A0 = c.Xs; g.lda = c.K;
        g.C = c.Cpart; g.ldc = c.LdetP;
        g.M = c.NP; g.N = c.LdetP; g.K = c.K; g.splitK = c.splitK; g.sCsplit = (long)c.NP * c.LdetP;
        {
            Prof pr(p, "gemm_wblur_fwd", sB);
            if (p->wblur_fp32) {
                g.B0 = c.Wt; g.ldb = c.LdetP;
                LAUNCH_OK(gemm32(p, sB, g));
            } else {
                g.ldb = c.K;
                g.B16 = c.W16; g.pB16 = (long)c.LdetP * c.K; g.sB16 = c.sW;
                g.A3 = c.Xs16; g.pA3 = (long)c.NP * c.K;
                g.bscale = c.bscale; g.segLinP = c.LinP; g.segChunks = (c.LinP + 1023) / 1024;
                g.klist = c.klF; g.klistStride = c.klFs;
                LAUNCH_OK(launch_gemm_nt_f16x2_cc(sB, g));
            }
        }
        if (hand_over && c.ymat16) {
            Prof pr(p, "ymat16_from_cpart", sB);
            LAUNCH_OK(launch_ymat16_from_cpart(sB, c.Cpart, (long)c.NP * c.LdetP, c.splitK, c.ymat16, (long)c.NP * c.LdetP, c.amax, c.NP,
                                               c.P * c.S * c.aout, c.Ldet, c.LdetP));
        } else {
            Prof pr(p, "y_from_cpart", sB);
            LAUNCH_OK(launch_y_from_cpart(sB, c.Cpart, (long)c.NP * c.LdetP, c.splitK, y + c.yoff, c.P * c.S, c.Ldet,
                                          c.aout, c.LdetP));
        }
    }
    if (chain(p, sB, s)) return 1;
    return 0;
}

int adjoint_dev(surfh_plan *p, const float *y, float *x, bool ref, bool handed_over = false) {
    hipStream_t s = p->stream;
    hipStream_t sB = (p->overlap && p->stream2) ? p->stream2 : s;
    if (chain(p, s, sB)) return 1;
    float *const acc = (!ref && p->gcube) ? p->gcube : p->cube;
    if (acc == p->cube) {
        Prof pr(p, "fill_zero");
        LAUNCH_OK(launch_fill_zero(s, p->cube, (long)p->NBP * p->NAP * p->LP));
    }
    auto prepare = [&](Channel &c) -> int {
        const bool f16 = c.W16 != nullptr;
        if (handed_over && f16 && c.ymat16) return 0;
        {
            Prof pr(p, "ymat_from_y", sB);
            LAUNCH_OK(launch_ymat_from_y(sB, y + c.yoff, c.ymat, c.P * c.S, c.Ldet, c.aout, c.LdetP, f16 ? c.pmax : nullptr,
                                         f16 ? c.amax : nullptr, c.NP));
        }
        if (f16 && !p->wblur_fp32)
            LAUNCH_OK(launch_split_rows2h(sB, c.ymat, c.amax, c.ymat16, c.NP, c.LdetP, (long)c.NP * c.LdetP));
        return 0;
    };
    auto gemm_args = [&](Channel &c) {
        GemmArgs g;
        g.A0 = c.ymat; g.lda = c.LdetP;
        g.C = c.Xs; g.ldc = c.K;
        g.M = c.NP; g.N = c.K; g.K = c.LdetP;
        if (p->wblur_fp32) {
            g.B0 = c.W; g.ldb = c.K;
        } else if (c.W16) {
            g.K = (c.Ldet + 31) / 32 * 32;
            g.ldb = c.LdetP;
            g.B16 = c.Wt16; g.pB16 = (long)c.LdetP * c.K; g.sB16 = c.sW; g.amax = c.amax;
            g.A3 = c.ymat16; g.pA3 = (long)c.NP * c.LdetP;
            g.klist = c.klA; g.klistStride = c.klAs;
            if (c.klA && c.permA) { g.permP = c.permA; g.permLin = c.LinP; }
        }
        return g;
    };
    std::vector<char> gemm_done(p->ch.size(), 0);
    if (p->gemm_grouped && !p->wblur_fp32 && !p->verify) {
        std::vector<GemmArgs> ga;
        std::vector<size_t> gc;
        for (size_t ci = 0; ci <= p->ch.size(); ++ci) {
            const bool last = ci == p->ch.size();
            if (!last) {
                Channel &c = p->ch[ci];
                if (c.bsum || !c.W16 || (ref && !c.has_ref)) continue;
                if (prepare(c)) return 1;
                ga.push_back(gemm_args(c)); gc.push_back(ci);
            }
            if (!ga.empty() && (last || (int)ga.size() == GEMM_GROUP_MAX)) {
                {
                    Prof pr(p, "gemm_wblur_adj", sB);
                    LAUNCH_OK(launch_gemm_nt_f16x2_cc_group(sB, ga.data(), (int)ga.size()));
                }
                for (size_t i : gc) gemm_done[i] = 1;
                ga.clear(); gc.clear();
            }
        }
    }
    for (size_t ci = 0; ci < p->ch.size(); ++ci) {
        Channel &c = p->ch[ci];
        if (ref && !c.has_ref) return fail("adjoint_ref needs the gridding_t tables (gt_*) in the channel descriptor");
        if (c.bsum) {
            {
                Prof pr(p, "y_transpose");
                LAUNCH_OK(launch_cube_to_lam_inner(s, y + c.yoff, c.Xs + c.shift, 0, c.Lin, 1, c.P * c.S * c.aout, 1, c.LinP));
            }
            Prof pr(p, ref ? "spmm_degrid_ref" : "spmm_scatter_adj");
            if (p->verify)
                LAUNCH_OK(launch_spmm_rows_f64acc(s, ref ? c.adjRef.t : c.adjT.t, c.Xs, acc, c.nlam, 1));
            else if (!ref && c.adjT.g.NG)
                LAUNCH_OK(launch_spmm_group_scatter(s, c.adjT.g, c.Xs, acc, c.nlam));
            else
                LAUNCH_OK(launch_spmm_rows(s, ref ? c.adjRef.t : c.adjT.t, c.Xs, acc, c.nlam, 1));
            continue;
        }
        if (!gemm_done[ci]) {
            if (prepare(c)) return 1;
            const GemmArgs g = gemm_args(c);
            Prof pr(p, "gemm_wblur_adj", sB);
            if (p->wblur_fp32 || !c.W16) LAUNCH_OK(gemm32(p, sB, g));
            else LAUNCH_OK(launch_gemm_nt_f16x2_cc(sB, g));
        }
        if (chain(p, sB, s)) return 1;
        {
            Prof pr(p, ref ? "spmm_degrid_ref" : "spmm_scatter_adj");
            if (p->verify)
                LAUNCH_OK(launch_spmm_rows_f64acc(s, ref ? c.adjRef.t : c.adjT.t, c.Xs, acc, c.nlam, 1));
            else if (!ref && c.adjT.g.NG)
                LAUNCH_OK(launch_spmm_group_scatter(s, c.adjT.g, c.Xs, acc, c.nlam));
            else
                LAUNCH_OK(launch_spmm_rows(s, ref ? c.adjRef.t : c.adjT.t, c.Xs, acc, c.nlam, 1));
        }
    }
    if (adjoint_tail(p, acc, true)) return 1;
    if (p->spec_out) return 0;
    if (p->T > 0) {
        if (irfft2_planes(p, p->mhat, p->maps_pad, p->T)) return 1;
        Prof pr(p, "unpad_planes");
        LAUNCH_OK(launch_unpad_planes(s, p->maps_pad, x, p->T, p->Na, p->Nb, p->NAP, p->NBP));
    } else if (prod_capable(p)) {
        ProdOperand po;
        po.prod = p->sotf; po.sign = -1.f; po.scale = p->pn_fold_prior ? (float)p->pl_mu : 1.f;
        if (p->pn_fold_prior && p->pl_mu_reg != 0.0 && p->pl_mu != 0.0) {
            po.add = p->mhat; po.add_w = (float)(p->pl_mu_reg / p->pl_mu);
        }
        float *const out = p->pn_native ? x : p->cube;
        if (irfft2_cube(p, p->spec, out, false, false, &po)) return 1;
        if (!p->pn_native) {
            const long pl = (long)p->Na * p->Nb;
            if (p->Lown < p->Lc) LAUNCH_OK(launch_fill_zero(s, x, (long)p->Lc * pl));
            Prof pr(p, "cube_transpose");
            for (auto &g : p->segs)
                LAUNCH_OK(launch_cube_from_lam_inner(s, p->cube + g.coff, x, g.start, g.len, p->Na, p->Nb, p->NAP, p->LP));
        }
    } else if (p->pn_native) {
        if (irfft2_cube(p, p->mhat, x)) return 1;
    } else {
        if (irfft2_cube(p, p->mhat, p->cube)) return 1;
        const long pl = (long)p->Na * p->Nb;
        if (p->Lown < p->Lc) LAUNCH_OK(launch_fill_zero(s, x, (long)p->Lc * pl));
        Prof pr(p, "cube_transpose");
        for (auto &g : p->segs)
            LAUNCH_OK(launch_cube_from_lam_inner(s, p->cube + g.coff, x, g.start, g.len, p->Na, p->Nb, p->NAP, p->LP));
    }
    return 0;
}

bool normal_hand_over(const surfh_plan *p) {
    static const bool fused = [] { const char *e = getenv("SURFH_NORMAL_FUSED"); return !(e && e[0] == '0'); }();
    return fused && !p->verify && !p->wblur_fp32;
}

int normal_dev(surfh_plan *p, const float *d, float *q, double mu) {
    const bool ho = normal_hand_over(p);
    if (forward_dev(p, d, p->cg_y, ho)) return 1;
    if (adjoint_dev(p, p->cg_y, q, false, ho)) return 1;
    if (mu != 1.0) {
        Prof pr(p, "scale");
        LAUNCH_OK(launch_scale(p->stream, q, p->pn_native ? (long)p->NBP * p->NAP * p->LP : p->isize, (float)mu));
    }
    return 0;
}

int ensure_hessian(surfh_plan *p) {
    if (p->hth && p->mhat2) return 0;
    float *h = nullptr, *m2 = nullptr;
    if (dev_alloc(&h, (size_t)p->T * p->T * p->PL) || dev_alloc(&m2, (size_t)p->T * 2 * p->PL)) {
        hipFree(h);
        hipFree(m2);
        return 1;
    }
    const int rc = launch_wct_hessian(p->stream, p->sotf, p->tpl, h, p->T, p->PL, p->LP, p->ilv);
    if (rc != 0) {
        hipFree(h);
        hipFree(m2);
        return fail("launch_wct_hessian failed: %s", hipGetErrorString((hipError_t)rc));
    }
    p->hth = h;
    p->mhat2 = m2;
    return 0;
}

int ensure_cg(surfh_plan *p) {
    if (p->cg_x) return 0;
    const size_t n = std::max((size_t)p->isize, (size_t)2 * std::max(p->T, 0) * (size_t)p->PL);
    for (float **v : {&p->cg_x, &p->cg_r, &p->cg_d, &p->cg_q, &p->cg_b})
        if (dev_alloc(v, n)) return 1;
    return 0;
}

}

extern "C" {

const char *surfh_last_error(void) { return g_err.c_str(); }
int surfh_version(void) { return 100; }

int surfh_plan_destroy(surfh_plan *p) {
    if (!p) return 0;
    hipSetDevice(p->dev);
    if (p->stream) hipStreamSynchronize(p->stream);
    for (float *v : {p->sotf, p->tpl, p->mhat, p->spec, p->ycol, p->cube, p->ycol_maps, p->maps_pad, p->Fi, p->Gi, p->Gf,
                     p->Ff, p->GiT, p->GfT, p->Cma, p->Sma, p->Gc, p->Gs, p->Cf, p->Sf, p->io_cube, p->hth, p->mhat2, p->gcube, p->io_x, p->io_y, p->cg_x, p->cg_r, p->cg_d, p->cg_q, p->cg_b, p->cg_y, p->cg_qm, p->cg_dd})
        hipFree(v);
    hipFree(p->h2img);
// ... 142 lines not shown
                const double *src = cfg->sotf ? cfg->sotf + ((size_t)p->planes[l] * p->Na + a) * nkb * 2 : nullptr;
                for (int k = 0; k < nkb; ++k) {
                    const float vr = src ? (float)src[2 * k] : 1.f, vi = src ? (float)src[2 * k + 1] : 0.f;
                    if (p->ilv) {
                        row[((size_t)k * LP + l) * 2] = vr;
                        row[((size_t)k * LP + l) * 2 + 1] = vi;
                    } else {
                        row[(size_t)k * LP + l] = vr;
                        row[((size_t)p->KBP + k) * LP + l] = vi;
                    }
                }
            }
            if (p->ilv) {
                if (hipMemcpy(p->sotf + (size_t)a * p->KBP * LP * 2, row.data(), (size_t)2 * p->KBP * LP * sizeof(float),
                              hipMemcpyHostToDevice) != hipSuccess)
                    return bail(fail("sotf upload failed"));
            } else
            for (int c = 0; c < 2; ++c)
                if (hipMemcpy(p->sotf + ((size_t)c * p->PL + (size_t)a * p->KBP) * LP, row.data() + (size_t)c * p->KBP * LP,
                              (size_t)p->KBP * LP * sizeof(float), hipMemcpyHostToDevice) != hipSuccess)
                    return bail(fail("sotf upload failed"));
        }
    }
    if (p->T > 0) {
        std::vector<float> t((size_t)p->T * LP, 0.f);
        for (int k = 0; k < p->T; ++k)
            for (int l = 0; l < p->Lown; ++l)
                if (p->planes[l] >= 0) t[(size_t)k * LP + l] = (float)cfg->templates[(size_t)k * p->Lc + p->planes[l]];
        if (dev_upload(&p->tpl, t)) return bail(1);
    }
    {
        std::vector<float> Fi, Gi, Gf, Ff, GiT, GfT;
        build_dft(p, Fi, Gi, Gf, Ff, GiT, GfT);
        if (dev_upload(&p->Fi, Fi) || dev_upload(&p->Gi, Gi) || dev_upload(&p->Gf, Gf) || dev_upload(&p->Ff, Ff) ||
            dev_upload(&p->GiT, GiT) || dev_upload(&p->GfT, GfT))
            return bail(1);
    }
    {
        const char *e = getenv("SURFH_DFT_DENSE");
        p->dense_dft = e && e[0] == '1';
        const char *e3 = getenv("SURFH_NO_FUSED_MIX");
        p->fuse_mix = !(e3 && e3[0] == '1');
        const char *e4 = getenv("SURFH_WBLUR_FP32");
        p->wblur_fp32 = e4 && e4[0] == '1';
        const char *e7 = getenv("SURFH_OVERLAP");
        p->overlap = e7 && e7[0] == '1';
        if (p->overlap && hipStreamCreateWithFlags(&p->stream2, hipStreamNonBlocking) != hipSuccess) return bail(fail("hipStreamCreate failed"));
        if (const char *ep = getenv("SURFH_OTF_PROD")) p->otf_prod = !(ep[0] == '0');
        const char *e15 = getenv("SURFH_GATHER_GROUPED");
        p->gather_grouped = !(e15 && e15[0] == '0');
        { const char *eg = getenv("SURFH_GEMM_GROUPED"); p->gemm_grouped = !(eg && eg[0] == '0'); }
        const char *e14 = getenv("SURFH_SCATTER_GROUPED");
        p->scatter_grouped = !(e14 && e14[0] == '0');
        const char *e12 = getenv("SURFH_GATHER_SORTED");
        p->gather_sorted = !(e12 && e12[0] == '0');
        const int ha = p->Na / 2 + 1, hb = p->Nb / 2 + 1;
        p->MPa = (ha + 127) / 128 * 128; p->KPa = (ha + 15) / 16 * 16;
        p->MPb = (hb + 127) / 128 * 128; p->KPb = (hb + 15) / 16 * 16;
        if (p->KPa > p->NAP || p->KPb > p->NBP || p->KPb > p->KBP) return bail(fail("cube too small for the folded DFT"));
        const double sa = 1.0 / std::sqrt((double)p->Na), sb = 1.0 / std::sqrt((double)p->Nb);
        std::vector<float> Cma((size_t)p->MPa * p->KPa, 0.f), Sma(Cma.size(), 0.f);
        for (int r = 0; r < ha; ++r)
            for (int k = 0; k < ha; ++k) {
                const double th = 2.0 * M_PI * (double)(((long)r * k) % p->Na) / (double)p->Na;
                Cma[(size_t)r * p->KPa + k] = (float)(std::cos(th) * sa);
                Sma[(size_t)r * p->KPa + k] = (float)(std::sin(th) * sa);
            }
        std::vector<float> Gc((size_t)p->MPb * p->KPb, 0.f), Gs(Gc.size(), 0.f), Cf(Gc.size(), 0.f), Sf(Gc.size(), 0.f);
        for (int b = 0; b < hb; ++b)
            for (int k = 0; k < hb; ++k) {
                const double th = 2.0 * M_PI * (double)(((long)b * k) % p->Nb) / (double)p->Nb;
                const double w = (k == 0 || (p->Nb % 2 == 0 && k == p->Nb / 2)) ? 1.0 : 2.0;
                Gc[(size_t)b * p->KPb + k] = (float)(w * std::cos(th) * sb);
                Gs[(size_t)b * p->KPb + k] = (float)(w * std::sin(th) * sb);
                Cf[(size_t)k * p->KPb + b] = (float)(std::cos(th) * sb);
                Sf[(size_t)k * p->KPb + b] = (float)(std::sin(th) * sb);
            }
        if (dev_upload(&p->Cma, Cma) || dev_upload(&p->Sma, Sma) || dev_upload(&p->Gc, Gc) || dev_upload(&p->Gs, Gs) ||
            dev_upload(&p->Cf, Cf) || dev_upload(&p->Sf, Sf))
            return bail(1);
        if (cfg->verify) {
            p->verify = true;
            p->dense_dft = true;
            p->fuse_mix = false;
            p->wblur_fp32 = true;
            p->overlap = false;
        }
        if (p->ax_a == 1 || p->ax_b == 1) {
            if ((p->ax_a == 1 && p->MPa != 128) || (p->ax_b == 1 && p->MPb != 128)) return bail(fail("internal: dft_h2 needs 128-row folded matrices"));
            std::vector<unsigned short> im(3 * DFT_H2_IMAGE_HALFS, 0);
            if (p->ax_a == 1) p->h2kA[0] = dft_h2_build_image(Cma.data(), Sma.data(), p->MPa, p->KPa, p->KPa, im.data());
            if (p->ax_b == 1) {
                p->h2kA[1] = dft_h2_build_image(Gc.data(), Gs.data(), p->MPb, p->KPb, p->KPb, im.data() + DFT_H2_IMAGE_HALFS);
                p->h2kA[2] = dft_h2_build_image(Cf.data(), Sf.data(), p->MPb, p->KPb, p->KPb, im.data() + 2 * DFT_H2_IMAGE_HALFS);
            }
            if (dev_upload(&p->h2img, im)) return bail(1);
        }
        if (p->h2) {
            const char *eaf = getenv("SURFH_ADJ_FUSED");
            if (!(eaf && eaf[0] == '0') && p->T >= 1 && p->T <= 4 && p->Na >= 127 && p->Na <= 255 && p->LP % 128 == 0) {
                if (otf_support(p, cfg)) return bail(1);
                const size_t npart = dft_h2_adjmix_part_floats(p->LP, p->Nb / 2 + 1, p->otf_nvalid);
                if (npart && dev_alloc(&p->adjmix_part, npart)) return bail(1);
            }
        }
        if (p->ct) {
            if (p->ax_a == 2 && dft_ct_plan_create(p->Na, &p->ctA)) return bail(fail("dft_ct plan (n_alpha = %d) failed", p->Na));
            if (p->ax_b == 2) {
                if (p->ax_a == 2 && p->Nb == p->Na) p->ctB = p->ctA;
                else if (dft_ct_plan_create(p->Nb, &p->ctB)) return bail(fail("dft_ct plan (n_beta = %d) failed", p->Nb));
            }
            if (p->ax_a == 2 && p->ax_b == 2 && p->T >= 1 && p->T <= 4 && otf_support(p, cfg)) return bail(1);
        }
        if (!p->ilv) p->dense_dft = true;
    }
    const size_t nspec = (size_t)2 * p->PL * LP, ncube = (size_t)p->NBP * p->NAP * LP;
    const size_t nycol = (size_t)2 * p->NAP * p->KBP * LP;
    const size_t nmhat = p->T > 0 ? (size_t)p->T * 2 * p->PL : nspec;
    const size_t nmaps = (size_t)std::max(p->T, 1) * p->PLc;
    const size_t nycm = (size_t)std::max(p->T, 1) * 2 * p->NAP * p->KBP;
    if (dev_alloc(&p->spec, nspec) || dev_alloc(&p->ycol, nycol) || dev_alloc(&p->cube, ncube) ||
        dev_alloc(&p->mhat, nmhat) || dev_alloc(&p->maps_pad, nmaps) || dev_alloc(&p->ycol_maps, nycm))
        return bail(1);
    hipMemset(p->spec, 0, nspec * sizeof(float));
    hipMemset(p->ycol, 0, nycol * sizeof(float));
    hipMemset(p->cube, 0, ncube * sizeof(float));
    hipMemset(p->mhat, 0, nmhat * sizeof(float));
    hipMemset(p->maps_pad, 0, nmaps * sizeof(float));
    hipMemset(p->ycol_maps, 0, nycm * sizeof(float));
    p->a_lo = p->b_lo = 1 << 30; p->a_hi = p->b_hi = 0;
    p->ch.resize(cfg->n_channels);
    long yoff = 0;
    for (int i = 0; i < cfg->n_channels; ++i) {
        if (build_channel(p, cfg->channels[i], &p->ch[i])) return bail(1);
        Channel &c = p->ch[i];
        c.yoff = yoff;
        yoff += c.ysize;
        if (c.bsum) continue;
        const bool f16 = !p->wblur_fp32;
        c.splitK = p->verify ? 1 : pick_split(c, cfg->split_k_forward, f16, p->n_cu);
        if (f16) {
            const long nw = (long)c.LdetP * c.K;
            const long nwv = ymat_from_y_waves(c.P * c.S, c.Ldet, c.aout);
            if (dev_alloc(&c.W16, (size_t)2 * nw) || dev_alloc(&c.Wt16, (size_t)2 * nw) || dev_alloc(&c.amax, (size_t)c.NP) ||
                dev_alloc(&c.pmax, (size_t)nwv) || dev_alloc(&c.ymat16, (size_t)2 * c.NP * c.LdetP) || dev_alloc(&c.Xs16, (size_t)2 * c.NP * c.K))
                return bail(1);
            hipMemset(c.pmax, 0, (size_t)nwv * sizeof(unsigned));
            hipMemset(c.amax, 0, (size_t)c.NP * sizeof(unsigned));
            hipMemset(c.Xs16, 0, (size_t)2 * c.NP * c.K * sizeof(unsigned short));
            std::vector<float> ones((size_t)c.nbs * ((c.LinP + 1023) / 1024) * c.NP, 1.f);
            if (dev_upload(&c.bscale, ones)) return bail(1);
            if (launch_split2h(p->stream, c.W, c.W16, nw, nw, c.sW) || launch_split2h(p->stream, c.Wt, c.Wt16, nw, nw, c.sW))
                return bail(fail("operand split failed"));
            const bool far_steps = !(cfg->exact & 1) && [] { const char *e = getenv("SURFH_WBLUR_FAR"); return !(e && e[0] == '0'); }();
            const double far_tol2 = [] { const char *e = getenv("SURFH_WBLUR_FAR_TOL2"); return std::ldexp(1.0, -(e ? atoi(e) : 10)); }();
            const int segChunks = (c.LinP + 1023) / 1024, KA = (c.Ldet + 31) / 32 * 32;
            if (far_steps && c.K / 32 <= 2048 && c.nbs * segChunks <= 64 && KA / 32 <= 2048) {
                std::vector<float> hw((size_t)nw);
                std::vector<int> kl;
                if (hipMemcpy(hw.data(), c.W, (size_t)nw * sizeof(float), hipMemcpyDeviceToHost) != hipSuccess) return bail(fail("copy failed"));
                build_klist(hw.data(), c.LdetP, c.K, c.K, c.LinP, segChunks, 1.0 / 256, far_tol2, &kl, &c.klFs, &c.ksteps[0], &c.ksteps[1]);
                if (c.ksteps[1] > 0 && dev_upload(&c.klF, kl)) return bail(1);
                if (hipMemcpy(hw.data(), c.Wt, (size_t)nw * sizeof(float), hipMemcpyDeviceToHost) != hipSuccess) return bail(fail("copy failed"));
                const bool perm = [] { const char *e = getenv("SURFH_WBLUR_PERM"); return !(e && e[0] == '0'); }();
                const int pP = perm && c.LinP % 64 == 0 && c.nbs >= 4 ? 4 : 0;
                build_klist(hw.data(), c.K, KA, c.LdetP, 0, 0, 1.0 / 256, far_tol2, &kl, &c.klAs, &c.ksteps[2], &c.ksteps[3], pP, c.LinP);
                if (c.ksteps[3] > 0) {
                    if (dev_upload(&c.klA, kl)) return bail(1);
                    c.permA = pP;
                }
            }
        }
        if (dev_alloc(&c.Cpart, (size_t)c.splitK * c.LdetP * c.NP)) return bail(1);
        hipMemset(c.Cpart, 0, (size_t)c.splitK * c.LdetP * c.NP * sizeof(float));
    }
    p->osize = yoff;
    if (p->a_hi <= p->a_lo) { p->a_lo = 0; p->a_hi = p->Na; }
    if (p->b_hi <= p->b_lo) { p->b_lo = 0; p->b_hi = p->Nb; }
    {
        const char *ear = getenv("SURFH_ALPHA_RANGE");
        if (ear && ear[0] == '0') { p->a_lo = 0; p->a_hi = p->Na; p->b_lo = 0; p->b_hi = p->Nb; }
        if (p->ilv && p->a_hi - p->a_lo < p->Na) {
            const size_t nyc = (size_t)2 * p->NAP * p->KBP * p->LP;
            if (dev_alloc(&p->ycol_adj, nyc)) return bail(1);
            if (hipMemset(p->ycol_adj, 0, nyc * sizeof(float)) != hipSuccess) return bail(fail("memset failed"));
        }
    }
    {
        const long npixrows = (long)p->NBP * p->NAP;
        bool exact_ok = !p->verify;
        {
            const char *ec = getenv("SURFH_ADJ_CLEAR");
            if (ec && ec[0] == '1') exact_ok = false;
        }
        std::vector<std::vector<uint8_t>> touched(p->ch.size());
        for (size_t ci = 0; ci < p->ch.size(); ++ci) {
            Channel &c = p->ch[ci];
            const std::vector<int64_t> &dst = c.adjT.host_dst;
            touched[ci].assign((size_t)npixrows, 0);
            const int nchunk = (c.nlam / 4 + 255) / 256;
            std::vector<uint32_t> mask(dst.size(), nchunk > 32 ? 0xFFFFFFFFu : 0u);
            std::vector<int2> ranges(dst.size(), make_int2(0, 0));
            for (size_t r = 0; r < dst.size(); ++r) {
                const long pix = (dst[r] - c.ws0a) / p->LP;
                if (pix < 0 || pix >= npixrows) return bail(fail("scatter table: bad destination"));
                touched[ci][pix] = 1;
                {
                    int lo = INT32_MAX, hi = INT32_MIN, covered = 0;
                    for (size_t cj = 0; cj < ci; ++cj) {
                        if (!touched[cj][pix]) continue;
                        const Channel &o = p->ch[cj];
                        const int a = std::max(o.ws0a, c.ws0a), b = std::min(o.ws0a + o.nlam, c.ws0a + c.nlam);
                        if (a >= b) continue;
                        if (covered && (a > hi || b < lo)) exact_ok = false;
                        lo = std::min(lo, a);
                        hi = std::max(hi, b);
                        covered = 1;
                    }
                    if (covered) ranges[r] = make_int2(lo - c.ws0a, hi - c.ws0a);
                }
                if (nchunk > 32) continue;
                for (size_t cj = 0; cj < ci; ++cj) {
                    if (!touched[cj][pix]) continue;
                    const Channel &o = p->ch[cj];
                    for (int j = 0; j < nchunk; ++j) {
                        const int lo = c.ws0a + 1024 * j, hi = std::min(c.ws0a + c.nlam, lo + 1024);
                        if (lo < o.ws0a + o.nlam && o.ws0a < hi) mask[r] |= 1u << j;
                    }
                }
            }
            {
                const char *ea0 = getenv("SURFH_SCATTER_RMW_ALL");
                if (ea0 && ea0[0] == '1') std::fill(mask.begin(), mask.end(), 0xFFFFFFFFu);
            }
            if (p->scatter_grouped) {
                const HostEll &h = c.adjT_host;
                std::vector<std::pair<size_t, size_t>> runs;
                for (size_t r = 0; r < h.rows.size();) {
                    size_t n = 1;
                    while (n < (size_t)SCATTER_G && r + n < h.rows.size() && h.dst[r + n] == h.dst[r + n - 1] + p->LP) ++n;
                    runs.push_back({r, n});
                    r += n;
                }
                if (upload_groups(h, runs, &mask, &c.adjT, SCATTER_G, &ranges)) return bail(1);
            }
            c.adjT_host = HostEll();
            if (dev_upload(&c.adjT.rmw, mask) || dev_upload(&c.adjT.rng, ranges)) return bail(1);
            c.adjT.t.rng = c.adjT.rng;
            const char *ea = getenv("SURFH_SCATTER_RMW_ALL");
            if (!(ea && ea[0] == '1')) c.adjT.t.rmw = c.adjT.rmw;
            c.adjT.host_dst.clear();
            c.adjT.host_dst.shrink_to_fit();
        }
        if (exact_ok && !p->ch.empty()) {
            const size_t ncube = (size_t)p->NBP * p->NAP * p->LP;
            if (dev_alloc(&p->gcube, ncube)) return bail(1);
            if (hipMemset(p->gcube, 0, ncube * sizeof(float)) != hipSuccess) return bail(fail("memset failed"));
        } else {
            for (auto &c : p->ch) {
                c.adjT.t.rng = nullptr;
                c.adjT.g.rng = nullptr;
            }
        }
    }
    if (dev_alloc(&p->io_x, (size_t)p->isize) || dev_alloc(&p->io_y, (size_t)p->osize) || dev_alloc(&p->cg_y, (size_t)p->osize) ||
        dev_alloc(&p->dscal, 8) || dev_alloc(&p->dscratch, 1024))
        return bail(1);
    if (hipDeviceSynchronize() != hipSuccess) return bail(fail("device error during plan creation: %s", hipGetErrorString(hipGetLastError())));
    *out = p;
    return 0;
}

int64_t surfh_isize(const surfh_plan *p) { return p ? p->isize : -1; }
int64_t surfh_osize(const surfh_plan *p) { return p ? p->osize : -1; }
void *surfh_stream(const surfh_plan *p) { return p ? (void *)p->stream : nullptr; }

int surfh_forward_dev(surfh_plan *p, const float *x, float *y) {
    if (!p) return fail("null plan");
    HIP_OK(hipSetDevice(p->dev));
    return forward_dev(p, x, y);
}
int surfh_adjoint_dev(surfh_plan *p, const float *y, float *x) {
    if (!p) return fail("null plan");
    HIP_OK(hipSetDevice(p->dev));
    return adjoint_dev(p, y, x, false);
}
int surfh_adjoint_ref_dev(surfh_plan *p, const float *y, float *x) {
    if (!p) return fail("null plan");
    HIP_OK(hipSetDevice(p->dev));
    return adjoint_dev(p, y, x, true);
}
int surfh_fwadj_dev(surfh_plan *p, const float *x, float *out) {
    if (!p) return fail("null plan");
    HIP_OK(hipSetDevice(p->dev));
    return normal_dev(p, x, out, 1.0);
}

static int host_call(surfh_plan *p, const float *in, long nin, float *outp, long nout, int which) {
    if (!p || !in || !outp) return fail("null argument");
    HIP_OK(hipSetDevice(p->dev));
    float *din = (which == 0 || which == 3) ? p->io_x : p->io_y;
    float *dout = (which == 0) ? p->io_y : p->io_x;
    if (which == 3) {
        if (ensure_cg(p)) return 1;
        dout = p->cg_q;
    }
    HIP_OK(hipMemcpyAsync(din, in, nin * sizeof(float), hipMemcpyHostToDevice, p->stream));
    int rc = 0;
    if (which == 0) rc = forward_dev(p, din, dout);
    else if (which == 1) rc = adjoint_dev(p, din, dout, false);
    else if (which == 2) rc = adjoint_dev(p, din, dout, true);
    else rc = normal_dev(p, din, dout, 1.0);
    if (rc) return rc;
    HIP_OK(hipMemcpyAsync(outp, dout, nout * sizeof(float), hipMemcpyDeviceToHost, p->stream));
    HIP_OK(hipStreamSynchronize(p->stream));
    return 0;
}

int surfh_forward(surfh_plan *p, const float *maps, float *y) { return host_call(p, maps, p ? p->isize : 0, y, p ? p->osize : 0, 0); }
// ... 673 lines not shown
    if (ensure_cg(p)) return 1;
    if (!p->cg_qm && (dev_alloc(&p->cg_qm, (size_t)p->isize) || dev_alloc(&p->cg_dd, (size_t)p->isize))) return 1;
    hipStream_t s = p->stream;
    const int L = p->Lc;
    const long npix = (long)p->Na * p->Nb, n = p->isize;
    float *r = p->cg_r, *m = p->cg_d, *d = p->cg_dd, *qd = p->cg_q, *qm = p->cg_qm;
    if (!p->pl_sc && dev_alloc(&p->pl_sc, (size_t)3 * L)) return 1;
    double *rr = p->pl_sc, *mqm = p->pl_sc + L;
    std::vector<float> hx;
    HIP_OK(hipMemcpyAsync(p->io_y, y, p->osize * sizeof(float), hipMemcpyHostToDevice, s));
    if (x0)
        HIP_OK(hipMemcpyAsync(p->cg_x, x0, n * sizeof(float), hipMemcpyHostToDevice, s));
    else
        LAUNCH_OK(launch_fill_zero(s, p->cg_x, n));
    LAUNCH_OK(launch_fill_zero(s, m, n));
    LAUNCH_OK(launch_fill_zero(s, qm, n));
    if (solver_setup(p, p->io_y, p->cg_x, mu, mu_reg)) return 1;
    *nit = 0;
    for (int it = 0;; ++it) {
        LAUNCH_OK(launch_mmmg_dir_planes(s, d, r, m, qm, L, npix, rr, mqm));
        double *gn = grad_norm + (size_t)it * L;
        HIP_OK(hipMemcpyAsync(gn, rr, L * sizeof(double), hipMemcpyDeviceToHost, s));
        HIP_OK(hipStreamSynchronize(s));
        double worst = 0.0;
        for (int l = 0; l < L; ++l) {
            gn[l] = std::sqrt(gn[l]);
            worst = std::max(worst, gn[l]);
        }
        if (const int rc = it > 0 ? callback_iterate(p, callback, user, it, grad_norm, p->cg_x, hx) : CB_GO_ON) {
            if (rc == CB_STOP) break;
            return 1;
        }
        if (it >= max_iter || worst < (double)npix * tol) break;
        if (normal_prior(p, d, qd, mu, mu_reg)) return 1;
        const bool fresh = refresh > 0 && it % refresh == 0;
        LAUNCH_OK(launch_mmmg_step_planes(s, p->cg_x, r, d, m, qm, qd, L, npix, mqm, fresh ? 0 : 1));
        if (fresh) {
            if (normal_prior(p, p->cg_x, qd, mu, mu_reg)) return 1;
            LAUNCH_OK(launch_residual(s, r, p->cg_b, qd, n));
        }
        *nit = it + 1;
    }
    HIP_OK(hipMemcpyAsync(x, p->cg_x, n * sizeof(float), hipMemcpyDeviceToHost, s));
    HIP_OK(hipStreamSynchronize(s));
    return 0;
}

int surfh_mmmg_planes(surfh_plan *p, const float *y, double mu, double mu_reg, const float *x0, int32_t max_iter, double tol,
                      int32_t refresh, float *x, double *grad_norm, int32_t *nit) {
    return surfh_mmmg_planes_cb(p, y, mu, mu_reg, x0, max_iter, tol, refresh, x, grad_norm, nit, nullptr, nullptr);
}

static int lmm_host(surfh_plan *p, const double *templates, int32_t T, int32_t L, const float *in, float *out, bool to_cube) {
    if (!p || !templates || !in || !out) return fail("null argument");
    if (T < 1 || L < 1) return fail("bad template shape");
    HIP_OK(hipSetDevice(p->dev));
    const long npix = (long)p->Na * p->Nb;
    std::vector<float> t((size_t)T * L);
    for (size_t i = 0; i < t.size(); ++i) t[i] = (float)templates[i];
    float *dt = nullptr, *dm = nullptr, *dc = nullptr;
    int rc = 0;
    auto done = [&](int r) { hipFree(dt); hipFree(dm); hipFree(dc); return r; };
    if (dev_upload(&dt, t) || dev_alloc(&dm, (size_t)T * npix) || dev_alloc(&dc, (size_t)L * npix)) return done(1);
    hipStream_t s = p->stream;
    if (to_cube) {
        if (hipMemcpyAsync(dm, in, (size_t)T * npix * sizeof(float), hipMemcpyHostToDevice, s) != hipSuccess) return done(fail("copy failed"));
        rc = launch_lmm_maps2cube(s, dm, dt, dc, T, L, npix);
        if (!rc) rc = (int)hipMemcpyAsync(out, dc, (size_t)L * npix * sizeof(float), hipMemcpyDeviceToHost, s);
    } else {
        if (hipMemcpyAsync(dc, in, (size_t)L * npix * sizeof(float), hipMemcpyHostToDevice, s) != hipSuccess) return done(fail("copy failed"));
        rc = launch_lmm_cube2maps(s, dc, dt, dm, T, L, npix);
        if (!rc) rc = (int)hipMemcpyAsync(out, dm, (size_t)T * npix * sizeof(float), hipMemcpyDeviceToHost, s);
    }
    if (!rc) rc = (int)hipStreamSynchronize(s);
    if (rc) return done(fail("lmm: %s", hipGetErrorString((hipError_t)rc)));
    return done(0);
}
int surfh_maps_to_cube(surfh_plan *p, const double *templates, int32_t T, int32_t L, const float *maps, float *cube) {
    return lmm_host(p, templates, T, L, maps, cube, true);
}
int surfh_cube_to_maps(surfh_plan *p, const double *templates, int32_t T, int32_t L, const float *cube, float *maps) {
    return lmm_host(p, templates, T, L, cube, maps, false);
}

int surfh_profile_enable(surfh_plan *p, int32_t on) {
    if (!p) return fail("null plan");
    p->prof = on != 0;
    return 0;
}
int surfh_profile_filter(surfh_plan *p, const char *prefix) {
    if (!p) return fail("null plan");
    p->prof_filter = prefix ? prefix : "";
    return 0;
}
int32_t surfh_profile_count(surfh_plan *p) {
    if (!p) return -1;
    hipSetDevice(p->dev);
    prof_collect(p);
    return (int32_t)p->acc_names.size();
}
int surfh_profile_get(surfh_plan *p, int32_t i, const char **name, int64_t *launches, double *ms) {
    if (!p || i < 0 || i >= (int32_t)p->acc_names.size()) return fail("bad profile index");
    auto &e = p->acc[p->acc_names[i]];
    *name = p->acc_names[i].c_str();
    *launches = e.first;
    *ms = e.second;
    return 0;
}
int surfh_profile_reset(surfh_plan *p) {
    if (!p) return fail("null plan");
    hipSetDevice(p->dev);
    prof_collect(p);
    p->acc.clear();
    p->acc_names.clear();
    return 0;
}

static int resolve(surfh_plan *p, const char *which, const float **ptr, int64_t dims[4]) {
    std::string w(which ? which : "");
    dims[0] = dims[1] = dims[2] = dims[3] = 1;
    *ptr = nullptr;
    if (w == "blurred" || w == "gcube") {
        *ptr = (w == "gcube" && p->gcube) ? p->gcube : p->cube; dims[0] = p->NBP; dims[1] = p->NAP; dims[2] = p->LP;
    } else if (w == "spec") {
        *ptr = p->spec;
        if (p->ilv) { dims[0] = p->KAP; dims[1] = p->KBP; dims[2] = p->LP; dims[3] = 2; }
        else { dims[0] = 2; dims[1] = p->KAP; dims[2] = p->KBP; dims[3] = p->LP; }
    } else if (w == "mhat" && p->T > 0) {
        *ptr = p->mhat; dims[0] = p->T; dims[1] = 2; dims[2] = p->KAP; dims[3] = p->KBP;
    } else if (w.rfind("xs:", 0) == 0 || w.rfind("xsinfo:", 0) == 0) {
        const bool info = w[2] == 'i';
        const int c = atoi(w.c_str() + (info ? 7 : 3));
        if (c < 0 || c >= (int)p->ch.size()) return fail("bad channel index");
        if (info) {
            dims[0] = p->ch[c].LinP; dims[1] = p->ch[c].shift; dims[2] = p->ch[c].nbs; dims[3] = p->ch[c].Lin;
        } else {
            Channel &ch = p->ch[c];
            if (ch.Xs16) {
                if (launch_dequant_f16x2(p->stream, ch.Xs16, (long)ch.NP * ch.K, ch.bscale, ch.Xs, ch.NP, ch.K, ch.LinP,
                                         (ch.LinP + 1023) / 1024))
                    return fail("dequant launch failed");
                if (hipStreamSynchronize(p->stream) != hipSuccess) return fail("dequant failed");
            }
            *ptr = p->ch[c].Xs; dims[0] = p->ch[c].NP; dims[1] = p->ch[c].bsum ? 1 : p->ch[c].nbs; dims[2] = p->ch[c].LinP;
        }
    } else if (w == "range") {
        dims[0] = p->a_lo; dims[1] = p->a_hi; dims[2] = p->b_lo; dims[3] = p->b_hi;
    } else if (w == "otf") {
        dims[0] = p->otf_vlist ? p->otf_nvalid : (long)(p->Nb / 2 + 1) * (p->LP / 128); dims[1] = (long)(p->Nb / 2 + 1) * (p->LP / 128);
    } else if (w == "ksteps") {
        for (auto &c : p->ch)
            for (int i = 0; i < 4; ++i) dims[i] += c.ksteps[i];
        for (int i = 0; i < 4; ++i) dims[i] -= 1;
    } else if (w == "info") {
        dims[0] = p->lo; dims[1] = p->hi; dims[2] = p->Lown; dims[3] = (int64_t)p->segs.size();
    } else {
        return fail("unknown debug buffer '%s'", w.c_str());
    }
    return 0;
}

int surfh_debug_dims(surfh_plan *p, const char *which, int64_t dims[4]) {
    if (!p) return fail("null plan");
    const float *ptr;
    return resolve(p, which, &ptr, dims);
}

int64_t surfh_debug_copy(surfh_plan *p, const char *which, float *out, int64_t cap) {
    if (!p || !out) return -1;
    const float *ptr = nullptr;
    int64_t d[4];
    if (resolve(p, which, &ptr, d) || !ptr) return -1;
    const int64_t n = d[0] * d[1] * d[2] * d[3];
    if (n > cap) {
        fail("capacity %lld < %lld", (long long)cap, (long long)n);
        return -1;
    }
    hipSetDevice(p->dev);
    hipStreamSynchronize(p->stream);
    if (hipMemcpy(out, ptr, n * sizeof(float), hipMemcpyDeviceToHost) != hipSuccess) return -1;
    return n;
}

int32_t surfh_klist_classify(const float *B, int32_t n, int32_t k, int64_t ldb, int32_t perm_p, int32_t perm_lin, int32_t *records,
                             int64_t capacity) {
    if (!B || !records || n < 1 || k < 32 || k % 32 || ldb < k) return -fail("surfh_klist_classify: bad arguments");
    if (perm_p && ((perm_p != 1 && perm_p != 2 && perm_p != 4 && perm_p != 8) || perm_lin < 1 || perm_lin % (256 / perm_p) || n % perm_lin))
        return -fail("surfh_klist_classify: bad tile shape");
    std::vector<int> kl;
    int stride = 0;
    long nn = 0, nf = 0;
    build_klist(B, n, k, ldb, 0, 0, 1.0 / 256, 1.0 / 1024, &kl, &stride, &nn, &nf, perm_p, perm_lin);
    if ((int64_t)kl.size() > capacity) return -fail("surfh_klist_classify: capacity too small");
    std::memcpy(records, kl.data(), kl.size() * sizeof(int));
    return (int32_t)(kl.size() / (size_t)stride);
}

static long g_selftest_ksteps[2] = {0, 0};
int surfh_gemm_selftest_ksteps(int64_t near_far[2]) {
    near_far[0] = g_selftest_ksteps[0]; near_far[1] = g_selftest_ksteps[1];
    return 0;
}

int surfh_gemm_selftest(int32_t device, int32_t M, int32_t N, int32_t K, int32_t split_k, const float *A,
                        const float *B, float *C) {
    HIP_OK(hipSetDevice(device));
    float *dA = nullptr, *dB = nullptr, *dC = nullptr;
    const int sk = std::max(1, (int)split_k);
    HIP_OK(hipMalloc((void **)&dA, (size_t)M * K * 4));
    HIP_OK(hipMalloc((void **)&dB, (size_t)K * N * 4));
    HIP_OK(hipMalloc((void **)&dC, (size_t)sk * M * N * 4));
    HIP_OK(hipMemcpy(dA, A, (size_t)M * K * 4, hipMemcpyHostToDevice));
    HIP_OK(hipMemcpy(dB, B, (size_t)K * N * 4, hipMemcpyHostToDevice));
    GemmArgs g;
    g.A0 = dA; g.lda = K; g.B0 = dB; g.ldb = N; g.C = dC; g.ldc = N;
    g.M = M; g.N = N; g.K = K; g.splitK = sk; g.sCsplit = (long)M * N;
    int rc;
    const char *mode = getenv("SURFH_SELFTEST_F16X2");
    if (mode && (mode[0] == '1' || mode[0] == '2')) {
        std::vector<float> bt((size_t)N * K);
        for (int k = 0; k < K; ++k)
            for (int n = 0; n < N; ++n) bt[(size_t)n * K + k] = B[(size_t)k * N + n];
        HIP_OK(hipMemcpy(dB, bt.data(), bt.size() * 4, hipMemcpyHostToDevice));
        g.ldb = K;
        unsigned short *dB16 = nullptr, *dA16 = nullptr;
        unsigned *dmax = nullptr;
        float amB = 0.f;
        for (float v : bt) amB = std::max(amB, std::fabs(v));
        std::vector<unsigned> rows((size_t)M, 0u);
        for (int m = 0; m < M; ++m) {
            float am = 0.f;
            for (int k = 0; k < K; ++k) am = std::max(am, std::fabs(A[(size_t)m * K + k]));
            memcpy(&rows[m], &am, 4);
        }
        HIP_OK(hipMalloc((void **)&dB16, bt.size() * 4));
        HIP_OK(hipMalloc((void **)&dmax, rows.size() * sizeof(unsigned)));
        HIP_OK(hipMalloc((void **)&dA16, (size_t)M * K * 4));
        HIP_OK(hipMemcpy(dmax, rows.data(), rows.size() * sizeof(unsigned), hipMemcpyHostToDevice));
        g.sB16 = gemm_f16x2_scale(amB); g.B16 = dB16; g.pB16 = (long)bt.size(); g.amax = dmax;
        rc = launch_split2h(nullptr, dB, dB16, (long)bt.size(), (long)bt.size(), g.sB16);
        if (rc == 0) rc = launch_split_rows2h(nullptr, dA, dmax, dA16, M, K, (long)M * K);
        g.A3 = dA16; g.pA3 = (long)M * K;
        int *dkl = nullptr;
        g_selftest_ksteps[0] = g_selftest_ksteps[1] = 0;
        if (mode[0] == '2') {
            std::vector<int> kl;
            const char *ep = getenv("SURFH_SELFTEST_PERM");
            const int lin = ep ? atoi(ep) : 0;
            if (lin > 0) { g.permP = 4; g.permLin = lin; }
            build_klist(bt.data(), N, K, K, 0, 0, 1.0 / 256, 1.0 / 1024, &kl, &g.klistStride, &g_selftest_ksteps[0], &g_selftest_ksteps[1], g.permP,
                        g.permLin);
            if (dev_upload(&dkl, kl)) return 1;
            g.klist = dkl;
        }
        if (rc == 0) rc = launch_gemm_nt_f16x2_cc(nullptr, g);
        if (rc == 0) rc = (int)hipDeviceSynchronize();
        hipFree(dkl);
        hipFree(dB16);
        hipFree(dmax);
        hipFree(dA16);
    } else {
        rc = launch_gemm_f32(nullptr, g);
    }
    if (rc == 0) rc = (int)hipDeviceSynchronize();
    std::vector<float> h((size_t)sk * M * N);
    if (rc == 0) rc = (int)hipMemcpy(h.data(), dC, h.size() * 4, hipMemcpyDeviceToHost);
    hipFree(dA); hipFree(dB); hipFree(dC);
    if (rc) return fail("gemm selftest failed: %s", hipGetErrorString((hipError_t)rc));
    for (size_t i = 0; i < (size_t)M * N; ++i) {
        float s = 0.f;
        for (int k = 0; k < sk; ++k) s += h[(size_t)k * M * N + i];
        C[i] = s;
    }
    return 0;
}

}
```

### surfh_amd/models.py

```python
from __future__ import annotations

import ctypes as C
from math import ceil
from typing import List, Optional, Sequence

import numpy as np

from . import _lib, instru
from .geometry import ChannelGeometry
from .linop import LinOp


def _ptr(t):
    if isinstance(t, int):
        return C.c_void_p(t)
    return C.c_void_p(t.data_ptr())


class Channel(ChannelGeometry):
    device = 0

    def _aux(self, key, wavel_axis, pointings, **opts):
        cache = self.__dict__.setdefault("_aux_ops", {})
        if key not in cache:
# ... 153 lines not shown

    def adjoint_ref(self, inarray):
        return self._host(self._L.surfh_adjoint_ref, inarray, self.osize, self.ishape)

    def fwadj(self, x):
        return self._host(self._L.surfh_fwadj, x, self.isize, self.ishape)

    def forward_dev(self, maps_t, y_t):
        _lib.check(self._L.surfh_forward_dev(self._plan, _ptr(maps_t), _ptr(y_t)))

    def adjoint_dev(self, y_t, maps_t):
        _lib.check(self._L.surfh_adjoint_dev(self._plan, _ptr(y_t), _ptr(maps_t)))

    def adjoint_ref_dev(self, y_t, maps_t):
        _lib.check(self._L.surfh_adjoint_ref_dev(self._plan, _ptr(y_t), _ptr(maps_t)))

    def normal_dev(self, d_t, q_t, mu: float = 1.0):
        _lib.check(self._L.surfh_normal_dev(self._plan, _ptr(d_t), _ptr(q_t), float(mu)))

    def spec_supported(self) -> bool:
        return bool(self._L.surfh_spec_supported(self._plan))

    @property
    def spec_size(self) -> int:
        return int(self._L.surfh_spec_size(self._plan))

    def to_spec_dev(self, x_t, xt_t):
        _lib.check(self._L.surfh_to_spec_dev(self._plan, _ptr(x_t), _ptr(xt_t)))

    def from_spec_dev(self, xt_t, x_t):
        _lib.check(self._L.surfh_from_spec_dev(self._plan, _ptr(xt_t), _ptr(x_t)))

    def forward_spec_dev(self, dt_t, y_t):
        _lib.check(self._L.surfh_forward_spec_dev(self._plan, _ptr(dt_t), _ptr(y_t)))

    def adjoint_spec_dev(self, y_t, qt_t, mu: float = 1.0, dt_t=None, mu_reg: float = 0.0):
        _lib.check(self._L.surfh_adjoint_spec_dev(self._plan, _ptr(y_t), _ptr(qt_t), float(mu), _ptr(dt_t) if dt_t is not None else None,
                                                  float(mu_reg)))

    def normal_spec_dev(self, dt_t, qt_t, mu: float = 1.0, mu_reg: float = 0.0):
        _lib.check(self._L.surfh_normal_spec_dev(self._plan, _ptr(dt_t), _ptr(qt_t), float(mu), float(mu_reg)))

    def prior_spec_add_dev(self, dt_t, qt_t, mu_reg: float):
        _lib.check(self._L.surfh_prior_spec_add_dev(self._plan, _ptr(dt_t), _ptr(qt_t), float(mu_reg)))

    def prior_add_dev(self, d_t, q_t, mu_reg: float):
        _lib.check(self._L.surfh_prior_add_dev(self._plan, _ptr(d_t), _ptr(q_t), float(mu_reg)))

    def dot_dev(self, a_t, b_t, n: int) -> float:
        out = C.c_double()
        _lib.check(self._L.surfh_dot_dev(self._plan, _ptr(a_t), _ptr(b_t), int(n), C.byref(out)))
        return out.value

    def cg_step_dev(self, x_t, r_t, d_t, q_t, n: int, rr: float) -> float:
        out = C.c_double()
        _lib.check(self._L.surfh_cg_step_dev(self._plan, _ptr(x_t), _ptr(r_t), _ptr(d_t), _ptr(q_t), int(n), float(rr),
                                             C.byref(out)))
        return out.value

    def cg_iter_dev(self, x_t, r_t, d_t, q_t, n: int, rr: float) -> float:
        out = C.c_double()
        _lib.check(self._L.surfh_cg_iter_dev(self._plan, _ptr(x_t), _ptr(r_t), _ptr(d_t), _ptr(q_t), int(n), float(rr), C.byref(out)))
        return out.value

    def cg_dir_dev(self, d_t, r_t, n: int, beta: float):
        _lib.check(self._L.surfh_cg_dir_dev(self._plan, _ptr(d_t), _ptr(r_t), int(n), float(beta)))

    def cg_begin_dev(self, r_t, n: int):
        _lib.check(self._L.surfh_cg_begin_dev(self._plan, _ptr(r_t), int(n)))

    def cg_iter_nosync_dev(self, x_t, r_t, d_t, q_t, n: int):
        _lib.check(self._L.surfh_cg_iter_nosync_dev(self._plan, _ptr(x_t), _ptr(r_t), _ptr(d_t), _ptr(q_t), int(n)))

    def cg_xupdate_nosync_dev(self, x_t, d_t, q_t, n: int):
        _lib.check(self._L.surfh_cg_xupdate_nosync_dev(self._plan, _ptr(x_t), _ptr(d_t), _ptr(q_t), int(n)))

    def cg_refresh_nosync_dev(self, r_t, b_t, q_t, d_t, n: int):
        _lib.check(self._L.surfh_cg_refresh_nosync_dev(self._plan, _ptr(r_t), _ptr(b_t), _ptr(q_t), _ptr(d_t), int(n)))

    def cg_trace(self, cap: int = 1 << 16) -> np.ndarray:
        out = np.zeros(cap, dtype=np.float64)
        n = self._L.surfh_cg_trace(self._plan, _lib.dptr(out), int(cap))
        if n < 0:
            raise RuntimeError("surfh_cg_trace failed")
        return out[:n].copy()

    def residual_dev(self, r_t, b_t, q_t, n: int):
        _lib.check(self._L.surfh_residual_dev(self._plan, _ptr(r_t), _ptr(b_t), _ptr(q_t), int(n)))

    def set_prior(self, gradient: str = "separated"):
        if gradient not in ("separated", "joint"):
            raise ValueError(f"gradient must be 'separated' or 'joint', not {gradient!r}")
        _lib.check(self._L.surfh_set_prior(self._plan, 1 if gradient == "joint" else 0))
        self._prior = gradient

    def get_prior(self) -> str:
        return getattr(self, "_prior", "separated")

    def cg(self, data, mu=1.0, mu_reg=0.0, x0=None, max_iter=10, tol=1e-12, refresh=50, callback=None):
        return _lib.solve(self, self._L.surfh_cg_cb, data, mu, mu_reg, x0, max_iter, tol, refresh, callback)

    def mmmg(self, data, mu=1.0, mu_reg=0.0, x0=None, max_iter=10, tol=1e-12, refresh=50, callback=None):
        return _lib.solve(self, self._L.surfh_mmmg, data, mu, mu_reg, x0, max_iter, tol, refresh, callback)

    def cubeTomaps(self, cube):
        cube = np.ascontiguousarray(np.asarray(cube, dtype=np.float32))
        tpl = np.ascontiguousarray(self.templates, dtype=np.float64)
        if cube.shape != (tpl.shape[1], self.ishape[-2], self.ishape[-1]):
            raise ValueError(f"cube shape {cube.shape} != {(tpl.shape[1], self.ishape[-2], self.ishape[-1])}")
        out = np.empty((tpl.shape[0],) + cube.shape[1:], dtype=np.float32)
        _lib.check(self._L.surfh_cube_to_maps(self._plan, _lib.dptr(tpl), tpl.shape[0], tpl.shape[1], _lib.fptr(cube), _lib.fptr(out)))
        return out.astype(np.float64)

    def mapsToCube(self, maps):
        tpl = np.ascontiguousarray(self.templates, dtype=np.float64)
        maps = np.ascontiguousarray(np.asarray(maps, dtype=np.float32).reshape((tpl.shape[0],) + tuple(self.ishape[-2:])))
        out = np.empty((tpl.shape[1],) + maps.shape[1:], dtype=np.float32)
        _lib.check(self._L.surfh_maps_to_cube(self._plan, _lib.dptr(tpl), tpl.shape[0], tpl.shape[1], _lib.fptr(maps), _lib.fptr(out)))
        return out.astype(np.float64)

    def real_data_janskySR_to_jansky(self, data):
        out = np.zeros_like(data)
        for k, ch in enumerate(self.channels):
            d = np.array(data[self._idx[k]: self._idx[k + 1]]).reshape(self.instrs_oshape[k])
            for s in range(self.instrs_oshape[k][1]):
                sl = ch.slicer.get_slit_slices(s)
                w = ch.slicer.get_slit_weights(s, sl)
                d[:, s, :, :] = d[:, s, :, :] * np.sum(w[0, 0, :]) * self.srfs[self.owned[k]]
            out[self._idx[k]: self._idx[k + 1]] = d.ravel()
        return out

    def profile_filter(self, prefix=None):
        _lib.check(self._L.surfh_profile_filter(self._plan, prefix.encode() if prefix else None))

    def profile_enable(self, on=True):
        _lib.check(self._L.surfh_profile_enable(self._plan, 1 if on else 0))

    def profile_reset(self):
        _lib.check(self._L.surfh_profile_reset(self._plan))

    def profile(self) -> dict:
        n = self._L.surfh_profile_count(self._plan)
        out = {}
        for i in range(n):
            name, cnt, ms = C.c_char_p(), C.c_int64(), C.c_double()
            _lib.check(self._L.surfh_profile_get(self._plan, i, C.byref(name), C.byref(cnt), C.byref(ms)))
            out[name.value.decode()] = (cnt.value, ms.value)
        return out

    def debug_buffer(self, which: str) -> np.ndarray:
        dims = (C.c_int64 * 4)()
        _lib.check(self._L.surfh_debug_dims(self._plan, which.encode(), dims))
        shape = tuple(int(d) for d in dims)
        if which in ("info", "range", "ksteps", "otf") or which.startswith("xsinfo:"):
            return np.array(shape)
        while len(shape) > 1 and shape[-1] == 1:
            shape = shape[:-1]
        out = np.empty(int(np.prod(shape)), dtype=np.float32)
        n = self._L.surfh_debug_copy(self._plan, which.encode(), _lib.fptr(out), out.size)
        if n < 0:
            raise RuntimeError(self._L.surfh_last_error().decode())
        return out.reshape(shape)
```

Baseline: 358.2.

## Skip low-order fp16 split products per 16-row block on near k-steps

Extends the host-side k-step classification so that, for each near k-step, every 16-row block of the 256-column B tile gets a bit saying whether the two cross-term fp16 products are needed. This is decided by a per-row error budget against the spectral weight tolerances. The kernel stores these masks in LDS and, per wave, branches around the two low-order MFMAs. It also skips the DMA of the low B piece when neither 128-row half needs it. The wave-to-column mapping is remapped so the masks line up with the wave layout. The gain is less matrix-core and memory work on the blur GEMM, at the cost of extra scalar branches, LDS reads and mask storage, and accuracy now depends on the tolerance budget.

```diff
diff --git a/include/surfh_amd.h b/include/surfh_amd.h
--- a/include/surfh_amd.h
+++ b/include/surfh_amd.h
@@ -143,8 +143,11 @@
 int surfh_gemm_selftest(int32_t device, int32_t M, int32_t N, int32_t K, int32_t split_k,
                         const float *A, const float *B, float *C);
 int surfh_gemm_selftest_ksteps(int64_t near_far[2]);
+int surfh_gemm_selftest_kblocks(int64_t lo_all[2]);
 int32_t surfh_klist_classify(const float *B, int32_t n, int32_t k, int64_t ldb, int32_t perm_p, int32_t perm_lin,
                              int32_t *records, int64_t capacity);
+int32_t surfh_klist_classify_blocks(const float *B, int32_t n, int32_t k, int64_t ldb, int32_t perm_p, int32_t perm_lin,
+                                    int32_t *records, int64_t capacity);
 
 typedef struct surfh_tst surfh_tst;
 int surfh_tst_create(int32_t n_alpha, int32_t n_beta, int32_t n_lambda, int32_t n_templates, const double *templates,
diff --git a/surfh_amd/_lib.py b/surfh_amd/_lib.py
--- a/surfh_amd/_lib.py
+++ b/surfh_amd/_lib.py
@@ -50,7 +50,7 @@
     "surfh_adjoint_spec_dev", "surfh_normal_spec_dev", "surfh_prior_spec_add_dev", "surfh_set_prior", "surfh_dot_dev", "surfh_cg_step_dev", "surfh_cg_dir_dev", "surfh_cg_iter_dev", "surfh_residual_dev",
     "surfh_cg_begin_dev", "surfh_cg_iter_nosync_dev", "surfh_cg_xupdate_nosync_dev", "surfh_cg_refresh_nosync_dev", "surfh_cg_trace",
     "surfh_profile_enable", "surfh_profile_filter", "surfh_profile_count", "surfh_profile_get", "surfh_profile_reset", "surfh_debug_copy",
-    "surfh_debug_dims", "surfh_gemm_selftest", "surfh_gemm_selftest_ksteps", "surfh_klist_classify",
+    "surfh_debug_dims", "surfh_gemm_selftest", "surfh_gemm_selftest_ksteps", "surfh_gemm_selftest_kblocks", "surfh_klist_classify", "surfh_klist_classify_blocks",
     "surfh_shepard", "surfh_shepard_last_error",
 ]
 
@@ -132,6 +132,9 @@
     L.surfh_gemm_selftest_ksteps.argtypes = [C.POINTER(C.c_int64)]
     L.surfh_klist_classify.argtypes = [c_float_p, C.c_int32, C.c_int32, C.c_int64, C.c_int32, C.c_int32, C.POINTER(C.c_int32), C.c_int64]
     L.surfh_klist_classify.restype = C.c_int32
+    L.surfh_gemm_selftest_kblocks.argtypes = [C.POINTER(C.c_int64)]
+    L.surfh_klist_classify_blocks.argtypes = L.surfh_klist_classify.argtypes
+    L.surfh_klist_classify_blocks.restype = C.c_int32
     L.surfh_shepard.argtypes = [C.c_int32, C.POINTER(C.c_int64), vp, vp, vp, c_int32_p, c_int32_p, C.c_int32, vp, vp,
                                 c_float_p, c_float_p, C.c_float, C.c_float, C.c_float, C.c_float, vp, vp, C.c_int32, vp,
                                 c_float_p]
diff --git a/surfh_amd/csrc/gemm_cc16.hip b/surfh_amd/csrc/gemm_cc16.hip
--- a/surfh_amd/csrc/gemm_cc16.hip
+++ b/surfh_amd/csrc/gemm_cc16.hip
@@ -68,6 +68,10 @@
 __device__ __forceinline__ void cc2_dma(const char *base, unsigned off, unsigned l) {
     asm volatile("s_mov_b32 m0, %2\n\ts_nop 0\n\tglobal_load_lds_dwordx4 %0, %1" ::"v"(off), "s"(base), "s"(l) : "memory");
 }
+__device__ __forceinline__ void cc2_dma_if(const char *base, unsigned off, unsigned l, unsigned cond, int bit) {
+    asm volatile("s_bitcmp1_b32 %3, %4\n\ts_cbranch_scc0 1f\n\ts_mov_b32 m0, %2\n\ts_nop 0\n\tglobal_load_lds_dwordx4 %0, %1\n1:"
+                 ::"v"(off), "s"(base), "s"(l), "s"(cond), "n"(bit) : "memory", "scc");
+}
 
 #define CC_MFMA_DRAIN() asm volatile("s_nop 15\n\ts_nop 15\n\ts_nop 7" ::: "memory")
 
@@ -76,10 +80,16 @@
 template <int U, int N, bool DMA, bool FAR>
 __device__ __forceinline__ void cc16_slot(f32x4v (&acc)[4][8], f16x8 (&A)[4][2], const f16x8 (&Bc)[2][2], f16x8 (&Bn)[2][2], unsigned ran,
                                           unsigned rbn, const char *ka, const char *kb, long pA2, long pB2, const unsigned (&offA)[2],
-                                          const unsigned (&offB)[2], unsigned ls) {
+                                          const unsigned (&offB)[2], unsigned ls, unsigned lo, unsigned dlo) {
     constexpr int i = N / 6, jj = (N / 3) & 1, j = 2 * U + jj, p = N % 3;
-    if constexpr (!(CC_EXP & 4) && (!FAR || p == 2))
-        asm volatile("v_mfma_f32_16x16x32_f16 %0, %1, %2, %0" : "+v"(acc[i][j]) : "v"(A[i][p == 0 ? 1 : 0]), "v"(Bc[jj][p == 1 ? 1 : 0]));
+    if constexpr (!(CC_EXP & 4) && p == 2)
+        asm volatile("v_mfma_f32_16x16x32_f16 %0, %1, %2, %0" : "+v"(acc[i][j]) : "v"(A[i][0]), "v"(Bc[jj][0]));
+    if constexpr (!(CC_EXP & 4) && !FAR && p == 0)
+        asm volatile("s_bitcmp1_b32 %1, %2\n\ts_cbranch_scc0 1f\n\t"
+                     "v_mfma_f32_16x16x32_f16 %0, %3, %4, %0\n\tv_mfma_f32_16x16x32_f16 %0, %5, %6, %0\n1:"
+                     : "+v"(acc[i][j])
+                     : "s"(lo), "n"(2 * U + jj), "v"(A[i][1]), "v"(Bc[jj][0]), "v"(A[i][0]), "v"(Bc[jj][1])
+                     : "scc");
     if constexpr (N < 4 && !(CC_EXP & 2)) {
         constexpr int jn = 2 * ((U + 1) & 3) + (N >> 1), q = N & 1;
         if constexpr (!FAR || q == 0)
@@ -92,28 +102,29 @@
     constexpr int d = (U == 3 && N % 3 != 2 && N < 12) ? N - N / 3 : -1;
     if constexpr (DMA && d >= 0 && !(CC_EXP & 1) && (!FAR || d < 4)) {
         constexpr int q = d >> 2, i2 = (d >> 1) & 1;
-        if constexpr (d & 1) cc2_dma(kb + q * pB2, offB[i2], ls + (unsigned)((q * PIECE + (BM + i2 * 128) * BK) * 2));
+        if constexpr ((d & 1) && q == 1) cc2_dma_if(kb + q * pB2, offB[i2], ls + (unsigned)((q * PIECE + (BM + i2 * 128) * BK) * 2), dlo, i2);
+        else if constexpr (d & 1) cc2_dma(kb + q * pB2, offB[i2], ls + (unsigned)((q * PIECE + (BM + i2 * 128) * BK) * 2));
         else cc2_dma(ka + q * pA2, offA[i2], ls + (unsigned)((q * PIECE + i2 * 128 * BK) * 2));
     }
 }
 template <int U, bool DMA, bool FAR, int N = 0>
 __device__ __forceinline__ void cc16_unit(f32x4v (&acc)[4][8], f16x8 (&A)[4][2], const f16x8 (&Bc)[2][2], f16x8 (&Bn)[2][2], unsigned ran,
                                           unsigned rbn, const char *ka, const char *kb, long pA2, long pB2, const unsigned (&offA)[2],
-                                          const unsigned (&offB)[2], unsigned ls) {
+                                          const unsigned (&offB)[2], unsigned ls, unsigned lo, unsigned dlo) {
     if constexpr (N < 24) {
         if constexpr (U == 0 && N == 18 && !(CC_EXP & 2)) {
             if constexpr (FAR) asm volatile("s_waitcnt lgkmcnt(3)" : "+v"(A[3][0]), "+v"(A[3][1]));
             else asm volatile("s_waitcnt lgkmcnt(5)" : "+v"(A[3][0]), "+v"(A[3][1]));
         }
-        cc16_slot<U, N, DMA, FAR>(acc, A, Bc, Bn, ran, rbn, ka, kb, pA2, pB2, offA, offB, ls);
-        cc16_unit<U, DMA, FAR, N + 1>(acc, A, Bc, Bn, ran, rbn, ka, kb, pA2, pB2, offA, offB, ls);
+        cc16_slot<U, N, DMA, FAR>(acc, A, Bc, Bn, ran, rbn, ka, kb, pA2, pB2, offA, offB, ls, lo, dlo);
+        cc16_unit<U, DMA, FAR, N + 1>(acc, A, Bc, Bn, ran, rbn, ka, kb, pA2, pB2, offA, offB, ls, lo, dlo);
     }
 }
 #define CC16_WAITB(n_, B_)                                                                                              \
     asm volatile("s_waitcnt lgkmcnt(" #n_ ")" : "+v"(B_[0][0]), "+v"(B_[1][0]), "+v"(B_[0][1]), "+v"(B_[1][1]))
 
 constexpr int CC2_MAXLIST = 2048;
-constexpr size_t LDS3_BYTES = LDS2_BYTES + (size_t)CC2_MAXLIST * sizeof(int);
+constexpr size_t LDS3_BYTES = LDS2_BYTES + (size_t)CC2_MAXLIST * sizeof(int) + (size_t)CC2_MAXLIST * sizeof(unsigned short);
 
 struct GemmGroup {
     GemmArgs g[GEMM_GROUP_MAX];
@@ -132,6 +143,7 @@
     const GemmArgs g = grp.g[gi];
     unsigned char *sctab = reinterpret_cast<unsigned char *>(lds + 2 * STAGE);
     int *klds = reinterpret_cast<int *>(sctab + CC2_MAXSEG * BM);
+    unsigned short *kmlds = reinterpret_cast<unsigned short *>(klds + CC2_MAXLIST);
     const int tid = threadIdx.x, lane = tid & 63, wave = __builtin_amdgcn_readfirstlane(tid >> 6);
     const int Q = g.permP ? BN / g.permP : BN, tilesL = g.permP ? g.permLin / Q : 0, ncol = g.permP ? g.N / g.permLin : 0;
     const int tilesM = (g.M + BM - 1) / BM, tilesN = g.permP ? (ncol + g.permP - 1) / g.permP * tilesL : (g.N + BN - 1) / BN, tiles = tilesM * tilesN;
@@ -154,7 +166,10 @@
         const int f0 = (int)((long)NF * sk / g.splitK), f1 = (int)((long)NF * (sk + 1) / g.splitK);
         nnear = __builtin_amdgcn_readfirstlane(a1 - a0);
         nfar = __builtin_amdgcn_readfirstlane(f1 - f0);
-        for (int e = tid; e < nnear; e += 512) klds[e] = kl[2 + a0 + e];
+        for (int e = tid; e < nnear; e += 512) {
+            klds[e] = kl[2 + a0 + e];
+            kmlds[e] = g.klistMasks ? (unsigned short)kl[2 + NN + NF + a0 + e] : (unsigned short)0xFFFF;
+        }
         for (int e = tid; e < nfar; e += 512) klds[nnear + e] = kl[2 + NN + f0 + e];
         if (bs) nseg = (g.K / g.segLinP) * g.segChunks;
     } else {
@@ -168,6 +183,7 @@
         for (int e = tid; e < nnear; e += 512) {
             const int k = kbeg + e * BK;
             klds[e] = (k / BK) | (bs ? ((k / g.segLinP) * g.segChunks + (k % g.segLinP) / 1024) << 16 : 0);
+            kmlds[e] = 0xFFFF;
         }
     }
     for (int e = tid; e < nseg * BM; e += 512) {
@@ -193,9 +209,9 @@
     const char *baseB = cc2_uniform(reinterpret_cast<const char *>(g.B16 + (long)b * g.sB));
     const long pA2 = g.pA3 * 2, pB2 = g.pB16 * 2;
     const unsigned ldsw = (unsigned)(size_t)lds + (unsigned)(wave * 16 * BK * 2);
-    const unsigned kaddr = (unsigned)(size_t)klds;
+    const unsigned kaddr = (unsigned)(size_t)klds, kmaddr = (unsigned)(size_t)kmlds;
     const int l15 = lane & 15, kc = lane >> 4;
-    const int wm = wave >> 1, wn = wave & 1;
+    const int wm = wave >> 1, wn = (wave & 1) ^ (wave >> 2);
     f32x4v acc[4][8];
 #pragma unroll
     for (int i = 0; i < 4; ++i)
@@ -229,10 +245,11 @@
         constexpr bool FAR = decltype(far_tag)::value;
         constexpr int D = FAR ? 4 : 2;
         if (n <= 0) return;
-        int e[D];
+        int e[D], mk[D];
 #pragma unroll
         for (int s = 0; s < D; ++s) {
             e[s] = __builtin_amdgcn_readfirstlane(klds[lb + (s < n ? s : n - 1)]);
+            mk[s] = FAR ? 0 : __builtin_amdgcn_readfirstlane((int)kmlds[lb + (s < n ? s : n - 1)]);
             CC_DMA(FAR, e[s] & 0xFFFF, s);
         }
         if (FAR) asm volatile("s_waitcnt vmcnt(12)" ::: "memory");
@@ -289,17 +306,26 @@
                 }
                 seg = nseg_;
             }
-            unsigned ev;
-            asm volatile("ds_read_b32 %0, %1" : "=v"(ev) : "v"(kaddr + 4u * (unsigned)(lb + (kt + D < n ? kt + D : n - 1))));
+            unsigned ev, mv = 0;
+            {
+                const unsigned ke = (unsigned)(lb + (kt + D < n ? kt + D : n - 1));
+                asm volatile("ds_read_b32 %0, %1" : "=v"(ev) : "v"(kaddr + 4u * ke));
+                if (!FAR) asm volatile("ds_read_u16 %0, %1" : "=v"(mv) : "v"(kmaddr + 2u * ke));
+            }
             const char *kz = baseA;
             const unsigned ls2 = ldsw + stofs(FAR, kt & (D - 1));
-            cc16_unit<0, false, FAR>(acc, A, Bx, By, ra, rb, kz, kz, pA2, pB2, offA, offB, ls2);
-            asm volatile("s_waitcnt lgkmcnt(0)" : "+v"(By[0][0]), "+v"(By[1][0]), "+v"(By[0][1]), "+v"(By[1][1]), "+v"(ev));
+            const unsigned wlo = FAR ? 0u : ((unsigned)mk[0] >> (8 * wn)) & 0xFFu;
+#define CC16_UNIT(U_, DMA_, Bc_, Bn_, ka_, kb_) cc16_unit<U_, DMA_, FAR>(acc, A, Bc_, Bn_, ra, rb, ka_, kb_, pA2, pB2, offA, offB, ls2, wlo, dlo);
+            unsigned dlo = 3u;
+            CC16_UNIT(0, false, Bx, By, kz, kz)
+            asm volatile("s_waitcnt lgkmcnt(0)" : "+v"(By[0][0]), "+v"(By[1][0]), "+v"(By[0][1]), "+v"(By[1][1]), "+v"(ev), "+v"(mv));
             const int en = __builtin_amdgcn_readfirstlane((int)ev);
+            const int mn = FAR ? 0 : __builtin_amdgcn_readfirstlane((int)mv);
+            if (!FAR) dlo = (((unsigned)mn >> wave) & 1u) | (((unsigned)mn >> (wave + 8)) & 1u) << 1;
             const char *ka2 = baseA + (long)(en & 0xFFFF) * (BK * 2), *kb2 = baseB + (long)(en & 0xFFFF) * (BK * 2);
-            cc16_unit<1, false, FAR>(acc, A, By, Bx, ra, rb, kz, kz, pA2, pB2, offA, offB, ls2);
+            CC16_UNIT(1, false, By, Bx, kz, kz)
             CC16_WAITB(0, Bx);
-            cc16_unit<2, false, FAR>(acc, A, Bx, By, ra, rb, kz, kz, pA2, pB2, offA, offB, ls2);
+            CC16_UNIT(2, false, Bx, By, kz, kz)
             CC16_WAITB(0, By);
             if (FAR) asm volatile("s_waitcnt vmcnt(8)\n\ts_barrier" ::: "memory");
             else asm volatile("s_waitcnt vmcnt(0)\n\ts_barrier" ::: "memory");
@@ -307,12 +333,14 @@
                 const unsigned nx = stofs(FAR, (kt + 1) & (D - 1));
                 ra = ra0 + nx; rb = ra0 + fbd + nx;
             }
-            cc16_unit<3, true, FAR>(acc, A, By, Bx, ra, rb, ka2, kb2, pA2, pB2, offA, offB, ls2);
+            CC16_UNIT(3, true, By, Bx, ka2, kb2)
+#undef CC16_UNIT
             if (FAR) { CC16_WAITB(1, Bx); }
             else { CC16_WAITB(2, Bx); }
 #pragma unroll
-            for (int s = 0; s + 1 < D; ++s) e[s] = e[s + 1];
+            for (int s = 0; s + 1 < D; ++s) { e[s] = e[s + 1]; mk[s] = mk[s + 1]; }
             e[D - 1] = en;
+            mk[D - 1] = mn;
         }
         asm volatile("s_waitcnt vmcnt(0) lgkmcnt(0)" ::: "memory");
     };
@@ -407,7 +435,8 @@
     if ((double)(BM + 1) * (double)g.ldc * 4.0 >= 2147483648.0) return (int)hipErrorInvalidValue;
     if ((double)g.M * (double)g.lda * 2.0 >= 4294967296.0 || (double)g.N * (double)g.ldb * 2.0 >= 4294967296.0) return (int)hipErrorInvalidValue;
     if (g.klist) {
-        if (g.batch != 1 || g.klistStride < 2 + g.K / BK || g.K / BK > CC2_MAXLIST || g.K / BK > 0xFFFF) return (int)hipErrorInvalidValue;
+        if (g.batch != 1 || g.klistStride < (g.klistMasks ? 2 + 2 * (g.K / BK) : 2 + g.K / BK) || g.K / BK > CC2_MAXLIST || g.K / BK > 0xFFFF)
+            return (int)hipErrorInvalidValue;
         if (g.bscale && (g.K / g.segLinP) * g.segChunks > CC2_MAXSEG) return (int)hipErrorInvalidValue;
     } else {
         const int Kper = g.K / g.splitK;
diff --git a/surfh_amd/csrc/gemm_f32.h b/surfh_amd/csrc/gemm_f32.h
--- a/surfh_amd/csrc/gemm_f32.h
+++ b/surfh_amd/csrc/gemm_f32.h
@@ -24,6 +24,7 @@
     int segLinP = 0, segChunks = 0;
     const int *klist = nullptr;
     int klistStride = 0;
+    int klistMasks = 0;
     int permP = 0, permLin = 0;
 };
 
diff --git a/surfh_amd/csrc/plan.hip b/surfh_amd/csrc/plan.hip
--- a/surfh_amd/csrc/plan.hip
+++ b/surfh_amd/csrc/plan.hip
@@ -80,6 +80,8 @@
     float sW = 1.f;
     int *klF = nullptr, *klA = nullptr;
     int klFs = 0, klAs = 0;
+    int klMasks = 0;
+    long kblocks[4] = {0, 0, 0, 0};
     int permA = 0;
     long ksteps[4] = {0, 0, 0, 0};
     unsigned *amax = nullptr;
@@ -533,7 +535,7 @@
 }
 
 int build_klist(const float *B, int N, int K, long ldb, int segLinP, int segChunks, double tol1, double tol2, std::vector<int> *out,
-                int *stride, long *n_near, long *n_far, int permP = 0, int permLin = 0) {
+                int *stride, long *n_near, long *n_far, int permP = 0, int permLin = 0, long *blocks = nullptr) {
     const int Q = permP ? 256 / permP : 256, tilesL = permP ? permLin / Q : 0, ncol = permP ? N / permLin : 0;
     const int nb = K / 32, tilesN = permP ? (ncol + permP - 1) / permP * tilesL : (N + 255) / 256;
     auto brow = [&](int tn, int v) {
@@ -541,11 +543,12 @@
         const int c = (tn / tilesL) * permP + v / Q;
         return c < ncol ? c * permLin + (tn % tilesL) * Q + v % Q : -1;
     };
-    *stride = 2 + nb;
+    *stride = blocks ? 2 + 2 * nb : 2 + nb;
     out->assign((size_t)tilesN * *stride, 0);
     *n_near = *n_far = 0;
+    if (blocks) blocks[0] = blocks[1] = 0;
     std::vector<double> l1((size_t)256 * nb), l2((size_t)256 * nb), L1(256), L2(256), c1(256), c2(256), imp(nb);
-    std::vector<int> order(nb);
+    std::vector<int> order(nb), bmask(nb);
     std::vector<char> far(nb);
     for (int tn = 0; tn < tilesN; ++tn) {
         const int nr = 256;
@@ -588,14 +591,55 @@
             far[b] = 1;
             ++nf;
         }
-        if (nf < 8) { std::fill(far.begin(), far.end(), 0); nf = 0; }
+        if (nf < 8) {
+            std::fill(far.begin(), far.end(), 0);
+            std::fill(c1.begin(), c1.end(), 0.0);
+            std::fill(c2.begin(), c2.end(), 0.0);
+            nf = 0;
+        }
+        std::fill(bmask.begin(), bmask.end(), 0xFFFF);
+        if (blocks) {
+            for (int bl = 0; bl < 16; ++bl) {
+                const int r0 = bl * 16;
+                int nn = 0;
+                for (int b = 0; b < nb; ++b) {
+                    if (far[b]) continue;
+                    double m = 0.0;
+                    for (int r = r0; r < r0 + 16; ++r)
+                        if (L1[r] > 0.0) m = std::max(m, std::max(l1[(size_t)r * nb + b] / (L1[r] * tol1), std::sqrt(l2[(size_t)r * nb + b] / L2[r]) / tol2));
+                    imp[b] = m;
+                    order[nn++] = b;
+                }
+                std::stable_sort(order.begin(), order.begin() + nn, [&](int a, int b) { return imp[a] < imp[b]; });
+                double d1[16], d2[16];
+                for (int r = 0; r < 16; ++r) { d1[r] = c1[r0 + r]; d2[r] = c2[r0 + r]; }
+                for (int i = 0; i < nn; ++i) {
+                    const int b = order[i];
+                    bool ok = true;
+                    for (int r = 0; r < 16 && ok; ++r)
+                        ok = d1[r] + l1[(size_t)(r0 + r) * nb + b] <= tol1 * L1[r0 + r] && d2[r] + l2[(size_t)(r0 + r) * nb + b] <= tol2 * tol2 * L2[r0 + r];
+                    if (!ok) break;
+                    for (int r = 0; r < 16; ++r) { d1[r] += l1[(size_t)(r0 + r) * nb + b]; d2[r] += l2[(size_t)(r0 + r) * nb + b]; }
+                    bmask[b] &= ~(1 << bl);
+                }
+            }
+        }
         int *rec = out->data() + (size_t)tn * *stride;
         rec[0] = nb - nf; rec[1] = nf;
         int in = 2, ifar = 2 + nb - nf;
         for (int b = 0; b < nb; ++b) {
             const int k = b * 32;
             const int e = b | ((segLinP ? (k / segLinP) * segChunks + (k % segLinP) / 1024 : 0) << 16);
-            if (far[b]) rec[ifar++] = e; else rec[in++] = e;
+            if (far[b]) {
+                rec[ifar++] = e;
+            } else {
+                if (blocks) {
+                    rec[2 + nb + (in - 2)] = bmask[b];
+                    blocks[0] += __builtin_popcount(bmask[b]);
+                    blocks[1] += 16;
+                }
+                rec[in++] = e;
+            }
         }
         *n_near += nb - nf; *n_far += nf;
     }
@@ -1119,7 +1163,7 @@
                 g.B16 = c.W16; g.pB16 = (long)c.LdetP * c.K; g.sB16 = c.sW;
                 g.A3 = c.Xs16; g.pA3 = (long)c.NP * c.K;
                 g.bscale = c.bscale; g.segLinP = c.LinP; g.segChunks = (c.LinP + 1023) / 1024;
-                g.klist = c.klF; g.klistStride = c.klFs;
+                g.klist = c.klF; g.klistStride = c.klFs; g.klistMasks = c.klMasks;
                 LAUNCH_OK(launch_gemm_nt_f16x2_cc(sB, g));
             }
         }
@@ -1170,7 +1214,7 @@
             g.ldb = c.LdetP;
             g.B16 = c.Wt16; g.pB16 = (long)c.LdetP * c.K; g.sB16 = c.sW; g.amax = c.amax;
             g.A3 = c.ymat16; g.pA3 = (long)c.NP * c.LdetP;
-            g.klist = c.klA; g.klistStride = c.klAs;
+            g.klist = c.klA; g.klistStride = c.klAs; g.klistMasks = c.klMasks;
             if (c.klA && c.permA) { g.permP = c.permA; g.permLin = c.LinP; }
         }
         return g;
@@ -1619,19 +1663,24 @@
             if (dev_upload(&c.bscale, ones)) return bail(1);
             if (launch_split2h(p->stream, c.W, c.W16, nw, nw, c.sW) || launch_split2h(p->stream, c.Wt, c.Wt16, nw, nw, c.sW))
                 return bail(fail("operand split failed"));
-            const bool far_steps = !(cfg->exact & 1) && [] { const char *e = getenv("SURFH_WBLUR_FAR"); return !(e && e[0] == '0'); }();
+            const char *far_env = getenv("SURFH_WBLUR_FAR");
+            const bool far_steps = !(cfg->exact & 1) && !(far_env && far_env[0] == '0');
+            const bool far_blocks = !(far_env && far_env[0] == '1');
             const double far_tol2 = [] { const char *e = getenv("SURFH_WBLUR_FAR_TOL2"); return std::ldexp(1.0, -(e ? atoi(e) : 10)); }();
             const int segChunks = (c.LinP + 1023) / 1024, KA = (c.Ldet + 31) / 32 * 32;
             if (far_steps && c.K / 32 <= 2048 && c.nbs * segChunks <= 64 && KA / 32 <= 2048) {
                 std::vector<float> hw((size_t)nw);
                 std::vector<int> kl;
                 if (hipMemcpy(hw.data(), c.W, (size_t)nw * sizeof(float), hipMemcpyDeviceToHost) != hipSuccess) return bail(fail("copy failed"));
-                build_klist(hw.data(), c.LdetP, c.K, c.K, c.LinP, segChunks, 1.0 / 256, far_tol2, &kl, &c.klFs, &c.ksteps[0], &c.ksteps[1]);
+                c.klMasks = far_blocks ? 1 : 0;
+                build_klist(hw.data(), c.LdetP, c.K, c.K, c.LinP, segChunks, 1.0 / 256, far_tol2, &kl, &c.klFs, &c.ksteps[0], &c.ksteps[1], 0, 0,
+                            far_blocks ? &c.kblocks[0] : nullptr);
                 if (c.ksteps[1] > 0 && dev_upload(&c.klF, kl)) return bail(1);
                 if (hipMemcpy(hw.data(), c.Wt, (size_t)nw * sizeof(float), hipMemcpyDeviceToHost) != hipSuccess) return bail(fail("copy failed"));
                 const bool perm = [] { const char *e = getenv("SURFH_WBLUR_PERM"); return !(e && e[0] == '0'); }();
                 const int pP = perm && c.LinP % 64 == 0 && c.nbs >= 4 ? 4 : 0;
-                build_klist(hw.data(), c.K, KA, c.LdetP, 0, 0, 1.0 / 256, far_tol2, &kl, &c.klAs, &c.ksteps[2], &c.ksteps[3], pP, c.LinP);
+                build_klist(hw.data(), c.K, KA, c.LdetP, 0, 0, 1.0 / 256, far_tol2, &kl, &c.klAs, &c.ksteps[2], &c.ksteps[3], pP, c.LinP,
+                            far_blocks ? &c.kblocks[2] : nullptr);
                 if (c.ksteps[3] > 0) {
                     if (dev_upload(&c.klA, kl)) return bail(1);
                     c.permA = pP;
@@ -2611,6 +2660,10 @@
         for (auto &c : p->ch)
             for (int i = 0; i < 4; ++i) dims[i] += c.ksteps[i];
         for (int i = 0; i < 4; ++i) dims[i] -= 1;
+    } else if (w == "kblocks") {
+        for (auto &c : p->ch)
+            for (int i = 0; i < 4; ++i) dims[i] += c.kblocks[i];
+        for (int i = 0; i < 4; ++i) dims[i] -= 1;
     } else if (w == "info") {
         dims[0] = p->lo; dims[1] = p->hi; dims[2] = p->Lown; dims[3] = (int64_t)p->segs.size();
     } else {
@@ -2655,9 +2708,27 @@
     return (int32_t)(kl.size() / (size_t)stride);
 }
 
-static long g_selftest_ksteps[2] = {0, 0};
+int32_t surfh_klist_classify_blocks(const float *B, int32_t n, int32_t k, int64_t ldb, int32_t perm_p, int32_t perm_lin, int32_t *records,
+                                    int64_t capacity) {
+    if (!B || !records || n < 1 || k < 32 || k % 32 || ldb < k) return -fail("surfh_klist_classify_blocks: bad arguments");
+    if (perm_p && ((perm_p != 1 && perm_p != 2 && perm_p != 4 && perm_p != 8) || perm_lin < 1 || perm_lin % (256 / perm_p) || n % perm_lin))
+        return -fail("surfh_klist_classify_blocks: bad tile shape");
+    std::vector<int> kl;
+    int stride = 0;
+    long nn = 0, nf = 0, blocks[2];
+    build_klist(B, n, k, ldb, 0, 0, 1.0 / 256, 1.0 / 1024, &kl, &stride, &nn, &nf, perm_p, perm_lin, blocks);
+    if ((int64_t)kl.size() > capacity) return -fail("surfh_klist_classify_blocks: capacity too small");
+    std::memcpy(records, kl.data(), kl.size() * sizeof(int));
+    return (int32_t)(kl.size() / (size_t)stride);
+}
+
+static long g_selftest_ksteps[2] = {0, 0}, g_selftest_kblocks[2] = {0, 0};
 int surfh_gemm_selftest_ksteps(int64_t near_far[2]) {
     near_far[0] = g_selftest_ksteps[0]; near_far[1] = g_selftest_ksteps[1];
+    return 0;
+}
+int surfh_gemm_selftest_kblocks(int64_t lo_all[2]) {
+    lo_all[0] = g_selftest_kblocks[0]; lo_all[1] = g_selftest_kblocks[1];
     return 0;
 }
 
@@ -2701,14 +2772,16 @@
         if (rc == 0) rc = launch_split_rows2h(nullptr, dA, dmax, dA16, M, K, (long)M * K);
         g.A3 = dA16; g.pA3 = (long)M * K;
         int *dkl = nullptr;
-        g_selftest_ksteps[0] = g_selftest_ksteps[1] = 0;
+        g_selftest_ksteps[0] = g_selftest_ksteps[1] = g_selftest_kblocks[0] = g_selftest_kblocks[1] = 0;
         if (mode[0] == '2') {
             std::vector<int> kl;
             const char *ep = getenv("SURFH_SELFTEST_PERM");
             const int lin = ep ? atoi(ep) : 0;
             if (lin > 0) { g.permP = 4; g.permLin = lin; }
+            const char *ef = getenv("SURFH_WBLUR_FAR");
+            g.klistMasks = !(ef && ef[0] == '1');
             build_klist(bt.data(), N, K, K, 0, 0, 1.0 / 256, 1.0 / 1024, &kl, &g.klistStride, &g_selftest_ksteps[0], &g_selftest_ksteps[1], g.permP,
-                        g.permLin);
+                        g.permLin, g.klistMasks ? g_selftest_kblocks : nullptr);
             if (dev_upload(&dkl, kl)) return 1;
             g.klist = dkl;
         }
diff --git a/surfh_amd/models.py b/surfh_amd/models.py
--- a/surfh_amd/models.py
+++ b/surfh_amd/models.py
@@ -329,7 +329,7 @@
         dims = (C.c_int64 * 4)()
         _lib.check(self._L.surfh_debug_dims(self._plan, which.encode(), dims))
         shape = tuple(int(d) for d in dims)
-        if which in ("info", "range", "ksteps", "otf") or which.startswith("xsinfo:"):
+        if which in ("info", "range", "ksteps", "kblocks", "otf") or which.startswith("xsinfo:"):
             return np.array(shape)
         while len(shape) > 1 and shape[-1] == 1:
             shape = shape[:-1]
```

Measured after the change: 359.0, median of 6. No clear change (+0.2%).
